# HpWang-whu/YOHO

Measured on AMD Instinct MI355X. Metric: keypoints/sec (5000 kp x60 rot desc+YOHO-O), higher is better.
Workload: dtype fp16x2 split (2^-22-accurate products, fp32 accumulate); 1 GPU

## Files before the change

yoho_amd/csrc/gemmf.h:

```cpp
#pragma once
#include <hip/hip_runtime.h>
#include <type_traits>
#include "common.h"

namespace yoho {

typedef float floatx16 __attribute__((ext_vector_type(16)));
typedef float floatx4 __attribute__((ext_vector_type(4)));
typedef unsigned uintx4 __attribute__((ext_vector_type(4)));
typedef _Float16 halfx8 __attribute__((ext_vector_type(8)));
typedef const __attribute__((address_space(1))) void* gptr_t;
typedef __attribute__((address_space(3))) void* lptr_t;

constexpr int FG_STAGE = 32768;
constexpr int FG_LDS = 4 * FG_STAGE;

static const int FG_ORD_D[NIR_ORD] = {5, 4, 3, 3, 1};
static const int FG_ORD_R[NIR_ORD] = {4, 3, 1, 2, 0};
static const int FG_IR_BASE[5] = {0, 1, 10, 19, 35};
static const int FG_IR_D[5] = {1, 3, 3, 4, 5};

struct FGemmArgs {
    const char* A;
    const char* B;
    const float* bias;
    const float* res;
    float* out;
    long long a_off[NIR_ORD], b_off[NIR_ORD];
    int NT[NIR_ORD], MT[NIR_ORD], rot[NIR_ORD];
    int dim[NIR_ORD], qbase[NIR_ORD];
    int cin, cout, kppad, nT32;
    float descale;
    int* rflag;
    const unsigned* amax;
};

template <int I, int N, typename Fn>
__device__ __forceinline__ void sfor(Fn&& f) {
    if constexpr (I < N) {
        f(std::integral_constant<int, I>{});
        sfor<I + 1, N>(f);
    }
}

__device__ __forceinline__ floatx16 mfma_h(uintx4 a, uintx4 b, floatx16 c) {
    union { uintx4 u; halfx8 h; } ca, cb;
    ca.u = a; cb.u = b;
    return __builtin_amdgcn_mfma_f32_32x32x16_f16(ca.h, cb.h, c, 0, 0, 0);
}

__device__ __forceinline__ const char* uniform_ptr(const char* p) {
    const unsigned long long v = reinterpret_cast<unsigned long long>(p);
    const unsigned lo = __builtin_amdgcn_readfirstlane((unsigned)v), hi = __builtin_amdgcn_readfirstlane((unsigned)(v >> 32));
    return reinterpret_cast<const char*>(((unsigned long long)hi << 32) | lo);
}

template <int MI, int NJ>
__device__ __forceinline__ void zero_acc(floatx16 (&acc)[MI][NJ]) {
#pragma unroll
    for (int i = 0; i < MI; ++i)
#pragma unroll
        for (int j = 0; j < NJ; ++j)
#pragma unroll
            for (int e = 0; e < 16; ++e) acc[i][j][e] = 0.f;
}

__device__ __forceinline__ bool fg3_map(const FGemmArgs& a, int xcd, int slot, int& t, int& local, int& r) {
    int start = 0;
    for (int u = 0; u < NIR_ORD; ++u) {
        const int ru = (xcd + a.rot[u]) & 7;
        const int cnt = a.NT[u] > ru ? ((a.NT[u] - 1 - ru) / 8 + 1) * a.MT[u] : 0;
        if (slot < start + cnt) { t = u; local = slot - start; r = ru; return true; }
        start += cnt;
    }
    return false;
}

inline int fgemm_grid(const FGemmArgs& a, int per_tile) {
    int tot = 0;
    for (int x = 0; x < 8; ++x) {
        int n = 0;
        for (int t = 0; t < NIR_ORD; ++t) {
            const int r = (x + a.rot[t]) & 7;
            if (a.NT[t] > r) n += ((a.NT[t] - 1 - r) / 8 + 1) * a.MT[t] * per_tile;
        }
        tot = n > tot ? n : tot;
    }
    return 8 * tot;
}

enum { F2_NOSTORE = 0x100, F2_MIX = 0x200, F2_ST_SC1 = 0x400, F2_ST_NT = 0x800, F2_SPARSE4 = 0x1000, F2_SPARSE16 = 0x2000, F2_K32 = 0x4000 };

__device__ __forceinline__ size_t slab_off(int tile32, int q, int cout8, int o, int half, int kp32) {
    return (((((size_t)tile32 * G + q) * cout8 + (o >> 3)) * 2 + half) * TILE + kp32) * 4;
}

template <int MI, int NJ>
__device__ __forceinline__ void residual_start(floatx16 (&acc)[MI][NJ], int row0, int kp0, int jidx, int d, int qbase, const float* res, float descale,
                                               int cout, int nT32, int lane) {
    const float inv = 1.f / descale;
    const int half = lane >> 5, kp32 = lane & 31, cout8 = cout >> 3;
#pragma unroll
    for (int bi = 0; bi < NJ; ++bi) {
        const int tile32 = (kp0 >> 5) + bi;
#pragma unroll
        for (int ai = 0; ai < MI; ++ai) {
            const int rowb = row0 + ai * 32;
            const int iidx = rowb / cout, o0 = rowb - iidx * cout;
            const bool ok = tile32 < nT32 && iidx < d;
            const int q = qbase + iidx * d + jidx;
#pragma unroll
            for (int q4 = 0; q4 < 4; ++q4) {
                const size_t off = slab_off(tile32, q, cout8, o0 + q4 * 8 + half * 4, half, kp32);
                const floatx4 v = *reinterpret_cast<const floatx4*>(res + (ok ? off : 0)) * (ok ? inv : 0.f);
                acc[ai][bi][4 * q4 + 0] = v.x; acc[ai][bi][4 * q4 + 1] = v.y;
                acc[ai][bi][4 * q4 + 2] = v.z; acc[ai][bi][4 * q4 + 3] = v.w;
            }
        }
    }
}

template <int MI, int NJ>
__device__ __forceinline__ void coef_epilogue(const floatx16 (&acc)[MI][NJ], int row0, int kp0, int jidx, int d, int qbase, float* out, const float* bias,
                                              float descale, int cout, int nT32, int* rflag, int lane, int flags) {
    const int half = lane >> 5, kp32 = lane & 31, cout8 = cout >> 3;
    unsigned top = 0u;
#ifdef YOHO_EXPERIMENTS
    if ((flags & F2_SPARSE4) && (blockIdx.x >> 3) % 4 != 0) flags |= F2_NOSTORE;
    if ((flags & F2_SPARSE16) && (blockIdx.x >> 3) % 16 != 0) flags |= F2_NOSTORE;
    const __amdgpu_buffer_rsrc_t orsrc = __builtin_amdgcn_make_buffer_rsrc(out, 0, 0x7FFFFFFF, 0x00020000);
#endif
#pragma unroll
    for (int bi = 0; bi < NJ; ++bi) {
        const int tile32 = (kp0 >> 5) + bi;
        if (tile32 >= nT32) continue;
#pragma unroll
        for (int ai = 0; ai < MI; ++ai) {
            const int rowb = row0 + ai * 32;
            const int iidx = rowb / cout, o0 = rowb - iidx * cout;
            if (iidx >= d) continue;
            const int q = qbase + iidx * d + jidx;
#pragma unroll
            for (int q4 = 0; q4 < 4; ++q4) {
                const int o = o0 + q4 * 8 + half * 4;
                floatx4 val;
                val.x = acc[ai][bi][4 * q4 + 0]; val.y = acc[ai][bi][4 * q4 + 1];
                val.z = acc[ai][bi][4 * q4 + 2]; val.w = acc[ai][bi][4 * q4 + 3];
                val *= descale;
                if (d == 1) val += *reinterpret_cast<const floatx4*>(bias + o) * 7.745966692414834f;
                const size_t off = slab_off(tile32, q, cout8, o, half, kp32);
#ifdef YOHO_EXPERIMENTS
                if (flags & F2_ST_SC1) __builtin_amdgcn_raw_buffer_store_b128(__builtin_bit_cast(uintx4, val), orsrc, (int)(off * 4), 0, 16);
                else if (flags & F2_ST_NT) __builtin_amdgcn_raw_buffer_store_b128(__builtin_bit_cast(uintx4, val), orsrc, (int)(off * 4), 0, 2);
                else if (!(flags & F2_NOSTORE))
#endif
                *reinterpret_cast<floatx4*>(out + off) = val;
                top = max(max(top, __float_as_uint(val.x) & 0x7FFFFFFFu), __float_as_uint(val.y) & 0x7FFFFFFFu);
                top = max(max(top, __float_as_uint(val.z) & 0x7FFFFFFFu), __float_as_uint(val.w) & 0x7FFFFFFFu);
            }
        }
    }
    note_range_bits(rflag, top, FP16_MAX / HF_ASCALE);
}

__device__ __forceinline__ floatx4 mfma_h16(uintx4 a, uintx4 b, floatx4 c) {
    union { uintx4 u; halfx8 h; } ca, cb;
    ca.u = a; cb.u = b;
    return __builtin_amdgcn_mfma_f32_16x16x32_f16(ca.h, cb.h, c, 0, 0, 0);
}

inline bool fgemm_layer_k32(const FGemmArgs& a) { return a.cin >= 256 && a.cin % 64 == 0 && a.cout >= 256; }

template <int NJ, typename Extra>
__device__ __forceinline__ void row_products32(floatx4 (&accrow)[NJ], const uintx4& al, const uintx4& ah, const uintx4 (&bh)[NJ], const uintx4 (&bl)[NJ],
                                               Extra&& extra) {
    sfor<0, 3 * NJ>([&](auto mc) {
        constexpr int m = decltype(mc)::value, j = m % NJ, p = m / NJ;
        accrow[j] = mfma_h16(p == 0 ? al : ah, p == 1 ? bl[j] : bh[j], accrow[j]);
        __builtin_amdgcn_sched_barrier(0);
        extra(mc);
        __builtin_amdgcn_sched_barrier(0);
    });
}

template <int LOB, int MI, int NJ>
__device__ __forceinline__ void stage32_plain(floatx4 (&acc)[MI][NJ], const char* pa, const char* pb) {
    uintx4 bh[NJ], bl[NJ], al[2], ah[2];
#pragma unroll
    for (int j = 0; j < NJ; ++j) {
        bh[j] = *reinterpret_cast<const uintx4*>(pb + j * 256);
        bl[j] = *reinterpret_cast<const uintx4*>(pb + LOB + j * 256);
    }
    al[0] = *reinterpret_cast<const uintx4*>(pa + 16384);
    ah[0] = *reinterpret_cast<const uintx4*>(pa);
    sfor<0, MI>([&](auto ic) {
        constexpr int i = decltype(ic)::value;
        if constexpr (i + 1 < MI) {
            al[(i + 1) & 1] = *reinterpret_cast<const uintx4*>(pa + 16384 + (i + 1) * 256);
            ah[(i + 1) & 1] = *reinterpret_cast<const uintx4*>(pa + (i + 1) * 256);
        }
        row_products32(acc[i], al[i & 1], ah[i & 1], bh, bl, [](auto) {});
    });
}

template <int MI, int NJ>
__device__ __forceinline__ void zero_acc(floatx4 (&acc)[MI][NJ]) {
#pragma unroll
    for (int i = 0; i < MI; ++i)
#pragma unroll
        for (int j = 0; j < NJ; ++j) acc[i][j] = floatx4{0.f, 0.f, 0.f, 0.f};
}

template <bool TO_SLAB>
__device__ __forceinline__ void swap_rows16(floatx4& x, floatx4& y) {
    typedef unsigned uintx2 __attribute__((ext_vector_type(2)));
#pragma unroll
    for (int e = 0; e < 4; ++e) {
        uintx2 r = {__float_as_uint(x[e]), __float_as_uint(y[e])};
        if constexpr (TO_SLAB) {
            r = __builtin_amdgcn_permlane16_swap(r.x, r.y, false, false);
            r = __builtin_amdgcn_permlane32_swap(r.x, r.y, false, false);
        } else {
            r = __builtin_amdgcn_permlane32_swap(r.x, r.y, false, false);
            r = __builtin_amdgcn_permlane16_swap(r.x, r.y, false, false);
        }
        x[e] = __uint_as_float(r.x); y[e] = __uint_as_float(r.y);
    }
}

template <int MI, int NJ>
__device__ __forceinline__ void residual_start(floatx4 (&acc)[MI][NJ], int row0, int kp0, int jidx, int d, int qbase, const float* res, float descale,
                                               int cout, int nT32, int lane) {
    static_assert(NJ % 2 == 0, "pairs of 16-column tiles");
    const float inv = 1.f / descale;
    const int half = lane >> 5, kp32 = lane & 31, cout8 = cout >> 3;
#pragma unroll
    for (int bi = 0; bi < NJ; bi += 2) {
        const int tile32 = (kp0 >> 5) + (bi >> 1);
#pragma unroll
        for (int ai = 0; ai < MI; ++ai) {
            const int rowb = row0 + ai * 16;
            const int iidx = rowb / cout, o0 = rowb - iidx * cout;
            const bool ok = tile32 < nT32 && iidx < d;
            const int q = qbase + iidx * d + jidx;
            const size_t off0 = slab_off(tile32, q, cout8, o0 + half * 4, half, kp32), off1 = slab_off(tile32, q, cout8, o0 + 8 + half * 4, half, kp32);
            acc[ai][bi] = *reinterpret_cast<const floatx4*>(res + (ok ? off0 : 0)) * (ok ? inv : 0.f);
            acc[ai][bi + 1] = *reinterpret_cast<const floatx4*>(res + (ok ? off1 : 0)) * (ok ? inv : 0.f);
            swap_rows16<false>(acc[ai][bi], acc[ai][bi + 1]);
        }
    }
}

template <int MI, int NJ>
__device__ __forceinline__ void coef_epilogue(const floatx4 (&acc)[MI][NJ], int row0, int kp0, int jidx, int d, int qbase, float* out, const float* bias,
                                              float descale, int cout, int nT32, int* rflag, int lane, int flags) {
    static_assert(NJ % 2 == 0, "pairs of 16-column tiles");
    const int half = lane >> 5, kp32 = lane & 31, cout8 = cout >> 3;
    unsigned top = 0u;
#pragma unroll
    for (int bi = 0; bi < NJ; bi += 2) {
        const int tile32 = (kp0 >> 5) + (bi >> 1);
        if (tile32 >= nT32) continue;
#pragma unroll
        for (int ai = 0; ai < MI; ++ai) {
            const int rowb = row0 + ai * 16;
            const int iidx = rowb / cout, o0 = rowb - iidx * cout;
            if (iidx >= d) continue;
            const int q = qbase + iidx * d + jidx;
            floatx4 v[2] = {acc[ai][bi], acc[ai][bi + 1]};
            swap_rows16<true>(v[0], v[1]);
#pragma unroll
            for (int h8 = 0; h8 < 2; ++h8) {
                const int o = o0 + h8 * 8 + half * 4;
                floatx4 val = v[h8] * descale;
                if (d == 1) val += *reinterpret_cast<const floatx4*>(bias + o) * 7.745966692414834f;
#ifdef YOHO_EXPERIMENTS
                if (!(flags & F2_NOSTORE))
#endif
                *reinterpret_cast<floatx4*>(out + slab_off(tile32, q, cout8, o, half, kp32)) = val;
                top = max(max(top, __float_as_uint(val.x) & 0x7FFFFFFFu), __float_as_uint(val.y) & 0x7FFFFFFFu);
                top = max(max(top, __float_as_uint(val.z) & 0x7FFFFFFFu), __float_as_uint(val.w) & 0x7FFFFFFFu);
            }
        }
    }
    note_range_bits(rflag, top, FP16_MAX / HF_ASCALE);
}

void fgemm_fill_args(FGemmArgs& a, const Layer& L, const char* Bplanes, int kppad, int nT32, const float* res, float* out, int* rflag);
int launch_fgemm2(const FGemmArgs& a, int flags, hipStream_t s);
int launch_fgemm3(const FGemmArgs& a, int flags, hipStream_t s);
int fgemm2_init();

}
```

yoho_amd/csrc/gemmf.hip:

```cpp
#include <hip/hip_runtime.h>
#include <hip/hip_fp16.h>
#include <type_traits>
#include <vector>
#include <cmath>
#include <cstring>
#include <cstdlib>

#include "common.h"
#include "gemmf.h"

namespace yoho {

struct Frags {
    uintx4 ah[4], al[4], bh[4], bl[4];
};

template <int SUB, int R>
__device__ __forceinline__ void read_frag(const char* pa, const char* pb, Frags& f) {
    constexpr int t = R & 3;
    if constexpr (R < 4) f.al[t] = *reinterpret_cast<const uintx4*>(pa + (2 + SUB) * 8192 + t * 512);
    else if constexpr (R < 8) f.bh[t] = *reinterpret_cast<const uintx4*>(pb + (0 + SUB) * 8192 + t * 512);
    else if constexpr (R < 12) f.ah[t] = *reinterpret_cast<const uintx4*>(pa + (0 + SUB) * 8192 + t * 512);
    else f.bl[t] = *reinterpret_cast<const uintx4*>(pb + (2 + SUB) * 8192 + t * 512);
}

template <int SUB>
__device__ __forceinline__ void read_frags(const char* pa, const char* pb, Frags& f) {
    sfor<0, 16>([&](auto rc) { read_frag<SUB, decltype(rc)::value>(pa, pb, f); });
}

template <int U>
__device__ __forceinline__ void stage_unit(const char* srcA, const char* srcB, char* dst, int w, int lane16) {
    constexpr int p = U & 7;
    const int blk = p * 4 + w;
    const char* src = (U < 8 ? srcA : srcB) + blk * 1024;
    char* d = dst + (U < 8 ? 0 : FG_STAGE) + blk * 1024;
    __builtin_amdgcn_global_load_lds((gptr_t)(src + lane16), (lptr_t)d, 16, 0, 0);
}

__device__ __forceinline__ void stage_tile(const char* src, char* dst, int w, int lane) {
#pragma unroll
    for (int p = 0; p < 8; ++p) {
        const int blk = p * 4 + w;
        __builtin_amdgcn_global_load_lds((gptr_t)(src + blk * 1024 + lane * 16), (lptr_t)(dst + blk * 1024), 16, 0, 0);
    }
}

template <int RSUB, bool DMA>
__device__ __forceinline__ void substep(const Frags& f, floatx16 (&acc)[4][4], const char* ra, const char* rb, Frags& nf,
                                        const char* srcA, const char* srcB, char* dmadst, int w, int lane16) {
    sfor<0, 16>([&](auto gc) {
        constexpr int g = decltype(gc)::value;
        acc[g >> 2][g & 3] = mfma_h(f.al[g >> 2], f.bh[g & 3], acc[g >> 2][g & 3]);
        read_frag<RSUB, g>(ra, rb, nf);
        __builtin_amdgcn_sched_barrier(0);
    });
    sfor<0, 16>([&](auto gc) {
        constexpr int g = decltype(gc)::value;
        acc[g >> 2][g & 3] = mfma_h(f.ah[g >> 2], f.bl[g & 3], acc[g >> 2][g & 3]);
        if constexpr (DMA) {
            stage_unit<g>(srcA, srcB, dmadst, w, lane16);
            __builtin_amdgcn_sched_barrier(0);
        }
    });
    __builtin_amdgcn_sched_barrier(0);
    sfor<0, 16>([&](auto gc) {
        constexpr int g = decltype(gc)::value;
        acc[g >> 2][g & 3] = mfma_h(f.ah[g >> 2], f.bh[g & 3], acc[g >> 2][g & 3]);
    });
    __builtin_amdgcn_sched_barrier(0);
}

__global__ __launch_bounds__(256, 1) void fgemm_kernel(FGemmArgs a, int flags) {
    extern __shared__ __attribute__((aligned(16))) char smem[];
    const int tid = threadIdx.x, lane = tid & 63;
    const int w = __builtin_amdgcn_readfirstlane(tid >> 6);
    int t = 0, local = 0, r = 0;
    if (!fg3_map(a, blockIdx.x & 7, blockIdx.x >> 3, t, local, r)) return;
    const int d = a.dim[t];
    const int MT = a.MT[t], KS = d * a.cin / 32;
    const int cg = local / MT, mtile = local - cg * MT;
    const int ntile = r + 8 * cg;
    const char* Ag = a.A + a.a_off[t] + (size_t)mtile * KS * FG_STAGE;
    const char* Bg = a.B + a.b_off[t] + (size_t)ntile * KS * FG_STAGE;
    const int wm = w >> 1, wn = w & 1;
    const int lane16 = lane * 16;
    const int row0 = mtile * 256 + wm * 128;
    const int col0 = ntile * 256 + wn * 128;

    floatx16 acc[4][4];
    zero_acc(acc);

    const int lane_a = (lane >> 5) * 4096 + (wm * 128 + (lane & 31)) * 16;
    const int lane_b = FG_STAGE + (lane >> 5) * 4096 + (wn * 128 + (lane & 31)) * 16;

    stage_tile(Ag, smem, w, lane);
    stage_tile(Bg, smem + FG_STAGE, w, lane);
    if (KS > 1) {
        stage_tile(Ag + FG_STAGE, smem + 2 * FG_STAGE, w, lane);
        stage_tile(Bg + FG_STAGE, smem + 3 * FG_STAGE, w, lane);
    }
    if ((flags & EPI_RES) && row0 < d * a.cout) residual_start(acc, row0, col0 % a.kppad, col0 / a.kppad, d, a.qbase[t], a.res, a.descale, a.cout, a.nT32, lane);
    asm volatile("s_waitcnt vmcnt(0)" ::: "memory");
    __syncthreads();

    if (row0 >= d * a.cout) {
        for (int s = 0; s < KS; ++s) {
            asm volatile("s_waitcnt vmcnt(0)" ::: "memory");
            __syncthreads();
            const int s2 = s + 2 < KS ? s + 2 : KS - 1;
            char* cur = smem + (s & 1) * (2 * FG_STAGE);
            stage_tile(Ag + (size_t)s2 * FG_STAGE, cur, w, lane);
            stage_tile(Bg + (size_t)s2 * FG_STAGE, cur + FG_STAGE, w, lane);
        }
        asm volatile("s_waitcnt vmcnt(0)" ::: "memory");
        return;
    }
    Frags P, Q;
    read_frags<0>(smem + lane_a, smem + lane_b, P);
    for (int s = 0; s < KS; ++s) {
        char* cur = smem + (s & 1) * (2 * FG_STAGE);
        char* nxt = smem + ((s + 1) & 1) * (2 * FG_STAGE);
        substep<1, false>(P, acc, cur + lane_a, cur + lane_b, Q, nullptr, nullptr, nullptr, w, lane16);
        asm volatile("s_waitcnt vmcnt(0) lgkmcnt(0)" ::: "memory");
        __syncthreads();
        __builtin_amdgcn_sched_barrier(0);
        const int s2 = s + 2 < KS ? s + 2 : KS - 1;
        substep<0, true>(Q, acc, nxt + lane_a, nxt + lane_b, P, uniform_ptr(Ag + (size_t)s2 * FG_STAGE), uniform_ptr(Bg + (size_t)s2 * FG_STAGE),
                              cur, w, lane16);
    }
    asm volatile("s_waitcnt vmcnt(0)" ::: "memory");

    coef_epilogue(acc, row0, col0 % a.kppad, col0 / a.kppad, d, a.qbase[t], a.out, a.bias, a.descale, a.cout, a.nT32, a.rflag, lane, flags);
}

__global__ __launch_bounds__(256, 1) void fgemmk_kernel(FGemmArgs a, int flags) {
    extern __shared__ __attribute__((aligned(16))) char smem[];
    const int tid = threadIdx.x, lane = tid & 63;
    const int w = __builtin_amdgcn_readfirstlane(tid >> 6);
    int t = 0, local = 0, r = 0;
    if (!fg3_map(a, blockIdx.x & 7, blockIdx.x >> 3, t, local, r)) return;
    const int d = a.dim[t];
    const int MT = a.MT[t], KS = d * a.cin / 32;
    const int cg = local / MT, mtile = local - cg * MT;
    const int ntile = r + 8 * cg;
    const char* Ag = a.A + a.a_off[t] + (size_t)mtile * KS * FG_STAGE;
    const char* Bg = a.B + a.b_off[t] + (size_t)ntile * KS * FG_STAGE;
    const int wm = w >> 1, wn = w & 1;
    const int row0 = mtile * 256 + wm * 128, col0 = ntile * 256 + wn * 128;
    const bool rows_live = row0 < d * a.cout;
    const int lane_a = (lane >> 4) * 4096 + (wm * 128 + (lane & 15)) * 16;
    const int lane_b = FG_STAGE + (lane >> 4) * 4096 + (wn * 128 + (lane & 15)) * 16;

    floatx4 acc[8][8];
    zero_acc(acc);
    stage_tile(Ag, smem, w, lane);
    stage_tile(Bg, smem + FG_STAGE, w, lane);
    if (KS > 1) {
        stage_tile(Ag + FG_STAGE, smem + 2 * FG_STAGE, w, lane);
        stage_tile(Bg + FG_STAGE, smem + 3 * FG_STAGE, w, lane);
    }
    if ((flags & EPI_RES) && rows_live) residual_start(acc, row0, col0 % a.kppad, col0 / a.kppad, d, a.qbase[t], a.res, a.descale, a.cout, a.nT32, lane);
    asm volatile("s_waitcnt vmcnt(0)" ::: "memory");
    __syncthreads();
    for (int s = 0; s < KS; ++s) {
        char* cur = smem + (s & 1) * (2 * FG_STAGE);
        if (rows_live) stage32_plain<FG_STAGE / 2>(acc, cur + lane_a, cur + lane_b);
        asm volatile("s_waitcnt vmcnt(0) lgkmcnt(0)" ::: "memory");
        __syncthreads();
        __builtin_amdgcn_sched_barrier(0);
        if (s + 2 < KS) {
            stage_tile(uniform_ptr(Ag + (size_t)(s + 2) * FG_STAGE), cur, w, lane);
            stage_tile(uniform_ptr(Bg + (size_t)(s + 2) * FG_STAGE), cur + FG_STAGE, w, lane);
        }
    }
    if (rows_live) coef_epilogue(acc, row0, col0 % a.kppad, col0 / a.kppad, d, a.qbase[t], a.out, a.bias, a.descale, a.cout, a.nT32, a.rflag, lane, flags);
}

int fgemm_init() {
    HIPCHK(hipFuncSetAttribute(reinterpret_cast<const void*>(&fgemm_kernel), hipFuncAttributeMaxDynamicSharedMemorySize, FG_LDS));
    HIPCHK(hipFuncSetAttribute(reinterpret_cast<const void*>(&fgemmk_kernel), hipFuncAttributeMaxDynamicSharedMemorySize, FG_LDS));
    if (int rc = cgemm_init()) return rc;
    return fgemm2_init();
}

static long long pack_off(int t, int rows, int kdim) {
    long long off = 0;
    for (int u = 0; u < t; ++u) off += (long long)((FG_ORD_D[u] * rows + 255) / 256) * (FG_ORD_D[u] * kdim / 32) * FG_STAGE;
    return off;
}

size_t fgemm_planes_bytes(int kppad, int cin) { return (size_t)pack_off(NIR_ORD, kppad, cin); }

void fgemm_qinfo(int* qi ) {
    for (int t = 0; t < NIR_ORD; ++t) {
        const int r = FG_ORD_R[t], d = FG_IR_D[r];
        for (int m = 0; m < d; ++m)
            for (int j = 0; j < d; ++j) {
                int* p = qi + (FG_IR_BASE[r] + m * d + j) * 4;
                p[0] = t; p[1] = m; p[2] = j; p[3] = d;
            }
    }
}
void fgemm_plane_offsets(int kppad, int cin, long long* off ) {
    for (int t = 0; t < NIR_ORD; ++t) off[t] = pack_off(t, kppad, cin);
}

static inline unsigned short half_bits_h(float x) {
    const _Float16 h = (_Float16)x;
    unsigned short u;
    std::memcpy(&u, &h, 2);
    return u;
}

static unsigned char e4m3_bits(float x) {
    const unsigned sgn = std::signbit(x) ? 0x80u : 0u;
    const float a = std::fabs(x);
    if (!(a == a)) return 0x7F;
    if (a >= 464.f) return (unsigned char)(sgn | 0x7E);
    if (a < std::ldexp(1.f, -6)) {
        const int r = (int)std::nearbyint(std::ldexp(a, 9));
        return (unsigned char)(sgn | (r == 8 ? 0x08 : r));
    }
    int e;
    (void)std::frexp(a, &e);
    int r = (int)std::nearbyint(std::ldexp(a, 3 - (e - 1)));
    if (r == 16) { r = 8; ++e; }
    const int E = e - 1 + 7;
    if (E > 15 || (E == 15 && r - 8 > 6)) return (unsigned char)(sgn | 0x7E);
    return (unsigned char)(sgn | (E << 3) | (r - 8));
}
static inline float half_value_h(unsigned short u) {
    _Float16 h;
    std::memcpy(&h, &u, 2);
    return (float)h;
}

static inline size_t apack_index(int row, int k, int KS) {
    const int mtile = row >> 8, rr = row & 255, ks = k >> 5, sub = (k >> 4) & 1, kg = (k >> 3) & 1, e = k & 7;
    return ((size_t)mtile * KS + ks) * (FG_STAGE / 2) + ((size_t)(sub * 2 + kg) * 256 + rr) * 8 + e;
}
static inline void put_split(unsigned short* pack, size_t idx, float x) {
    const _Float16 hi = (_Float16)x;
    pack[idx] = half_bits_h(x);
    pack[idx + 8192] = half_bits_h(x - (float)hi);
}
static void fp8_correction_planes(const std::vector<unsigned short>& out, std::vector<unsigned short>& out8) {
    out8 = out;
    const size_t nblk = out.size() / (FG_STAGE / 2);
    for (size_t b = 0; b < nblk; ++b) {
        const unsigned short* src = out.data() + b * (FG_STAGE / 2);
        unsigned char* dst = reinterpret_cast<unsigned char*>(out8.data() + b * (FG_STAGE / 2) + 8192);
        for (int u = 0; u < 1024; ++u)
            for (int e = 0; e < 8; ++e) {
                dst[u * 16 + e] = e4m3_bits(half_value_h(src[u * 8 + e]) * 0.25f);
                dst[u * 16 + 8 + e] = e4m3_bits(half_value_h(src[8192 + u * 8 + e]) * 512.f);
            }
    }
}

int pack_fgemm_weights(const FourierBasis& fb, const float* W, int cin, int cout, std::vector<unsigned short>& out, float* descale,
                       std::vector<unsigned short>* out8) {
    if ((cout % 256 && cout != 32) || cin % 32) return -1;
    std::vector<float> what((size_t)60 * cout * cin);
    std::vector<double> coef(60 * NTAP);
    for (int r = 0; r < 5; ++r) {
        const int d = FG_IR_D[r];
        for (int i = 0; i < d; ++i)
            for (int m = 0; m < d; ++m)
                for (int k = 0; k < NTAP; ++k) coef[(FG_IR_BASE[r] + i * d + m) * NTAP + k] = fb.rho[r][fb.n0[k]][m * d + i];
    }
    float wmax = 0.f;
    for (int f = 0; f < 60; ++f)
        for (int o = 0; o < cout; ++o)
            for (int c = 0; c < cin; ++c) {
                const float* wk = W + ((size_t)o * cin + c) * NTAP;
                double acc = 0.0;
                for (int k = 0; k < NTAP; ++k) acc += (double)wk[k] * coef[f * NTAP + k];
                const float v = (float)acc;
                what[((size_t)f * cout + o) * cin + c] = v;
                wmax = std::fmax(wmax, std::fabs(v));
            }
    int ex = 0;
    if (wmax > 0.f && std::isfinite(wmax)) (void)std::frexp(wmax, &ex);
    const float wscale = std::ldexp(1.f, 10 - ex);
    *descale = 1.f / (wscale * HF_ASCALE);
    out.assign((size_t)pack_off(NIR_ORD, cout, cin) / 2, 0);
    for (int t = 0; t < NIR_ORD; ++t) {
        const int r = FG_ORD_R[t], d = FG_IR_D[r];
        unsigned short* base = out.data() + pack_off(t, cout, cin) / 2;
        for (int i = 0; i < d; ++i)
            for (int o = 0; o < cout; ++o)
                for (int m = 0; m < d; ++m) {
                    const float* src = &what[((size_t)(FG_IR_BASE[r] + i * d + m) * cout + o) * cin];
                    for (int c = 0; c < cin; ++c) put_split(base, apack_index(i * cout + o, m * cin + c, d * cin / 32), src[c] * wscale);
                }
    }
    if (out8) fp8_correction_planes(out, *out8);
    return 0;
}

int pack_cgemm_weights(const float* W, int cin, int cout, int ntaps, std::vector<unsigned short>& out, float* descale, std::vector<unsigned short>& out8) {
    if (cout % 256 || cin % 32) return -1;
    float wmax = 0.f;
    for (size_t i = 0; i < (size_t)cout * cin * ntaps; ++i) wmax = std::fmax(wmax, std::fabs(W[i]));
    int ex = 0;
    if (wmax > 0.f && std::isfinite(wmax)) (void)std::frexp(wmax, &ex);
    const float wscale = std::ldexp(1.f, 10 - ex);
    *descale = 1.f / (wscale * H2_ASCALE);
    const int KS = ntaps * cin / 32;
    out.assign((size_t)(cout / 256) * KS * (FG_STAGE / 2), 0);
    for (int o = 0; o < cout; ++o)
        for (int tap = 0; tap < ntaps; ++tap)
            for (int c = 0; c < cin; ++c) put_split(out.data(), apack_index(o, tap * cin + c, KS), W[((size_t)o * cin + c) * ntaps + tap] * wscale);
    fp8_correction_planes(out, out8);
    return 0;
}

void fgemm_fill_args(FGemmArgs& a, const Layer& L, const char* Bplanes, int kppad, int nT32, const float* res, float* out, int* rflag) {
    a.rflag = rflag; a.amax = nullptr;
    a.A = reinterpret_cast<const char*>(L.wpg); a.B = Bplanes; a.bias = L.bias; a.res = res; a.out = out;
    a.cin = L.cin; a.cout = L.cout; a.kppad = kppad; a.nT32 = nT32; a.descale = L.wpg_descale;
    static const int ROT[NIR_ORD] = {0, 0, 4, 4, 2};
    for (int t = 0; t < NIR_ORD; ++t) {
        a.a_off[t] = pack_off(t, L.cout, L.cin);
        a.b_off[t] = pack_off(t, kppad, L.cin);
        a.MT[t] = (FG_ORD_D[t] * L.cout + 255) / 256;
        a.NT[t] = FG_ORD_D[t] * kppad / 256;
        a.rot[t] = ROT[t];
        a.dim[t] = FG_ORD_D[t];
        a.qbase[t] = FG_IR_BASE[FG_ORD_R[t]];
    }
}

int launch_fgemm(const Layer& L, const char* Bplanes, int kppad, int nT32, const float* res, float* out, int flags, hipStream_t s, int* rflag,
                 FGemmBlocking blocking, const unsigned* amax) {
    FGemmArgs a;
    fgemm_fill_args(a, L, Bplanes, kppad, nT32, res, out, rflag);
    static const int dbg_gemm1 = [] { const char* e = experiment_env("YOHO_PARTI_DEBUG"); return (e && std::strstr(e, "gemm1")) ? 1 : 0; }();
    if (dbg_gemm1) blocking = FG_TILE256_W4;
    if (blocking == FG_TILE256_W8 && amax && L.wpg8) { a.amax = amax; a.A = reinterpret_cast<const char*>(L.wpg8); }
    const char* dbg = experiment_env("YOHO_FGEMM_DEBUG");
    if (fgemm_layer_k32(a) && !a.amax && !(dbg && std::strstr(dbg, "k16"))) flags |= F2_K32;
    if (blocking == FG_TILE256_W8) return launch_fgemm3(a, flags, s);
    if (blocking != FG_TILE256_W4) return launch_fgemm2(a, flags, s);
    if (flags & F2_K32) hipLaunchKernelGGL(fgemmk_kernel, dim3(fgemm_grid(a, 1)), dim3(256), FG_LDS, s, a, flags);
    else hipLaunchKernelGGL(fgemm_kernel, dim3(fgemm_grid(a, 1)), dim3(256), FG_LDS, s, a, flags);
    HIPCHK(hipGetLastError());
    return 0;
}

}
```

yoho_amd/csrc/gemmf2.hip:

```cpp
#include <hip/hip_runtime.h>
#include <cstdlib>
#include <cstring>
#include "common.h"
#include "gemmf.h"

namespace yoho {

constexpr int F2_BUF = 24576;
constexpr int F2_LDS = 3 * F2_BUF;
constexpr int F3_BUF = 32768;
constexpr int F3_LDS = 3 * F3_BUF;

struct Frags2 {
    uintx4 ah[4], al[4], bh[2], bl[2];
};

template <int LO, int R>
__device__ __forceinline__ void read_frag2(const char* pa, const char* pb, Frags2& f) {
    if constexpr (R < 4) f.al[R] = *reinterpret_cast<const uintx4*>(pa + 8192 + R * 512);
    else if constexpr (R < 6) f.bh[R - 4] = *reinterpret_cast<const uintx4*>(pb + (R - 4) * 512);
    else if constexpr (R < 10) f.ah[R - 6] = *reinterpret_cast<const uintx4*>(pa + (R - 6) * 512);
    else f.bl[R - 10] = *reinterpret_cast<const uintx4*>(pb + LO + (R - 10) * 512);
}
template <int LO>
__device__ __forceinline__ void read_frags2(const char* pa, const char* pb, Frags2& f) {
    sfor<0, 12>([&](auto rc) { read_frag2<LO, decltype(rc)::value>(pa, pb, f); });
}

struct Dma2 {
    static constexpr int NP = 6, LO = 4096;
    int la, lb, w;
    __device__ __forceinline__ Dma2(int w_, int lane) : la(w_ * 1024 + lane * 16), lb((w_ >> 1) * 4096 + (w_ & 1) * 1024 + lane * 16), w(w_) {}
    template <int U>
    __device__ __forceinline__ void piece(const char* srcA, const char* srcB, char* buf) const {
        if constexpr (U < 4) {
            constexpr int plane = U >> 1, kg = U & 1;
            __builtin_amdgcn_global_load_lds((gptr_t)(srcA + plane * 16384 + kg * 4096 + la), (lptr_t)(buf + plane * 8192 + kg * 4096 + w * 1024), 16, 0, 0);
        } else {
            constexpr int plane = U - 4;
            __builtin_amdgcn_global_load_lds((gptr_t)(srcB + plane * 16384 + lb), (lptr_t)(buf + 16384 + plane * 4096 + (w >> 1) * 2048 + (w & 1) * 1024), 16, 0, 0);
        }
    }
};
struct Dma3 {
    static constexpr int NP = 4, LO = 8192;
    int la, ldst;
    __device__ __forceinline__ Dma3(int w8, int lane) : la(w8 * 1024 + lane * 16), ldst(w8 * 1024) {}
    template <int U>
    __device__ __forceinline__ void piece(const char* srcA, const char* srcB, char* buf) const {
        constexpr int plane = U & 1;
        if constexpr (U < 2) __builtin_amdgcn_global_load_lds((gptr_t)(srcA + plane * 16384 + la), (lptr_t)(buf + plane * 8192 + ldst), 16, 0, 0);
        else __builtin_amdgcn_global_load_lds((gptr_t)(srcB + plane * 16384 + la), (lptr_t)(buf + 16384 + plane * 8192 + ldst), 16, 0, 0);
    }
};
template <typename Dma>
__device__ __forceinline__ void dma_step(const Dma& dm, const char* srcA, const char* srcB, char* buf) {
    sfor<0, Dma::NP>([&](auto uc) { dm.template piece<decltype(uc)::value>(srcA, srcB, buf); });
}

template <bool DMA, typename Dma>
__device__ __forceinline__ void step2(const Dma& dm, const Frags2& f, floatx16 (&acc)[4][2], const char* ra, const char* rb, Frags2& nf,
                                      const char* srcA, const char* srcB, char* dmabuf) {
    sfor<0, 8>([&](auto gc) {
        constexpr int g = decltype(gc)::value;
        acc[g >> 1][g & 1] = mfma_h(f.al[g >> 1], f.bh[g & 1], acc[g >> 1][g & 1]);
        read_frag2<Dma::LO, g>(ra, rb, nf);
        __builtin_amdgcn_sched_barrier(0);
    });
    sfor<0, 8>([&](auto gc) {
        constexpr int g = decltype(gc)::value;
        acc[g >> 1][g & 1] = mfma_h(f.ah[g >> 1], f.bl[g & 1], acc[g >> 1][g & 1]);
        if constexpr (g < 4) read_frag2<Dma::LO, 8 + g>(ra, rb, nf);
        else if constexpr (DMA) dm.template piece<g - 4>(srcA, srcB, dmabuf);
        __builtin_amdgcn_sched_barrier(0);
    });
    sfor<0, 8>([&](auto gc) {
        constexpr int g = decltype(gc)::value;
        acc[g >> 1][g & 1] = mfma_h(f.ah[g >> 1], f.bh[g & 1], acc[g >> 1][g & 1]);
        if constexpr (DMA && 4 + g < Dma::NP) dm.template piece<4 + g>(srcA, srcB, dmabuf);
        __builtin_amdgcn_sched_barrier(0);
    });
}

__host__ __device__ inline bool fg2_map(const FGemmArgs& a, int xcd, int slot, bool contiguous, int& t, int& local, int& r) {
    int cnt[NIR_ORD], ru[NIR_ORD];
    for (int u = 0; u < NIR_ORD; ++u) {
        ru[u] = (xcd + a.rot[u]) & 7;
        cnt[u] = a.NT[u] > ru[u] ? ((a.NT[u] - 1 - ru[u]) / 8 + 1) * a.MT[u] * 2 : 0;
    }
    const int L = cnt[0], S = cnt[1] + cnt[2] + cnt[3] + cnt[4];
    int list, idx;
    if (contiguous) { list = slot < L ? 0 : 1; idx = slot < L ? slot : slot - L; }
    else {
        const int P = L < S ? L : S;
        if (slot < 2 * P) { list = slot & 1; idx = slot >> 1; }
        else { list = L > S ? 0 : 1; idx = P + (slot - 2 * P); }
    }
    if (list == 0) {
        if (idx >= L) return false;
        t = 0; local = idx; r = ru[0];
        return true;
    }
    for (int u = 1; u < NIR_ORD; ++u) {
        if (idx < cnt[u]) { t = u; local = idx; r = ru[u]; return true; }
        idx -= cnt[u];
    }
    return false;
}

__device__ __forceinline__ size_t step_off(int ks) { return (size_t)(ks >> 1) * FG_STAGE + (size_t)(ks & 1) * 8192; }

template <int BUF, typename Dma>
__device__ __forceinline__ void ring_prologue(int KT, Dma&& dma) {
    dma(0, 0);
    dma(1, BUF);
    if (KT > 2) dma(2, 2 * BUF);
}

template <int BUF, int INFLIGHT, typename F, typename Step>
__device__ __forceinline__ void ring_pipelined(char* smem, const char* Ag, const char* Bg, int KT, int lane_a, int lane_b, F& P, Step&& step) {
    F Q;
    asm volatile("s_waitcnt lgkmcnt(0)" ::: "memory");
    __builtin_amdgcn_s_barrier();
    __builtin_amdgcn_sched_barrier(0);
    int cur = 0, nxt = BUF;
    int s = 0;
    auto run = [&](auto dma, const F& f, F& nf) {
        if constexpr (decltype(dma)::value) {
            step(dma, f, nf, smem + nxt + lane_a, smem + nxt + lane_b, uniform_ptr(Ag + step_off(s + 3)), uniform_ptr(Bg + step_off(s + 3)), smem + cur);
            asm volatile("s_waitcnt vmcnt(%0) lgkmcnt(0)" ::"n"(INFLIGHT) : "memory");
        } else {
            step(dma, f, nf, smem + nxt + lane_a, smem + nxt + lane_b, nullptr, nullptr, nullptr);
            asm volatile("s_waitcnt vmcnt(0) lgkmcnt(0)" ::: "memory");
        }
        __builtin_amdgcn_s_barrier();
        __builtin_amdgcn_sched_barrier(0);
        cur = nxt; nxt = nxt == 2 * BUF ? 0 : nxt + BUF; ++s;
    };
    constexpr std::true_type dma;
    constexpr std::false_type nodma;
    while (s + 4 < KT) {
        run(dma, P, Q);
        run(dma, Q, P);
    }
    if (KT >= 4) {
        run(dma, P, Q);
        run(nodma, Q, P);
    }
    run(nodma, P, Q);
    step(nodma, Q, P, smem + cur + lane_a, smem + cur + lane_b, nullptr, nullptr, nullptr);
}

template <int BUF, typename Dma>
__device__ __forceinline__ void ring_pipelined_idle(int KT, Dma&& dma) {
    __builtin_amdgcn_s_barrier();
    for (int s = 0; s + 1 < KT; ++s) {
        if (s + 3 < KT) dma(s + 3, (s % 3) * BUF);
        asm volatile("s_waitcnt vmcnt(0)" ::: "memory");
        __builtin_amdgcn_s_barrier();
    }
}

__global__ __launch_bounds__(256, 2) void fgemm2_kernel(FGemmArgs a, int flags) {
    extern __shared__ __attribute__((aligned(16))) char smem[];
    const int tid = threadIdx.x, lane = tid & 63;
    const int w = __builtin_amdgcn_readfirstlane(tid >> 6);
    int t = 0, local = 0, r = 0;
    if (!fg2_map(a, blockIdx.x & 7, blockIdx.x >> 3, (flags & F2_MIX) == 0, t, local, r)) return;
    const int d = a.dim[t];
    const int MT = a.MT[t], KS = d * a.cin / 32, KT = 2 * KS;
    const int nh = local & 1, pair = local >> 1;
    const int cg = pair / MT, mtile = pair - cg * MT;
    const int ntile = r + 8 * cg;
    const char* Ag = a.A + a.a_off[t] + (size_t)mtile * KS * FG_STAGE;
    const char* Bg = a.B + a.b_off[t] + (size_t)ntile * KS * FG_STAGE + nh * 2048;
    const int wm = w >> 1, wn = w & 1;
    const Dma2 dm(w, lane);
    const int lane_a = (lane >> 5) * 4096 + (wm * 128 + (lane & 31)) * 16;
    const int lane_b = 16384 + (lane >> 5) * 2048 + (wn * 64 + (lane & 31)) * 16;

    floatx16 acc[4][2];
    zero_acc(acc);
    auto dma = [&](int st, int buf) { dma_step(dm, Ag + step_off(st), Bg + step_off(st), smem + buf); };
    ring_prologue<F2_BUF>(KT, dma);
    const int row0 = mtile * 256 + wm * 128, colbase = ntile * 256 + nh * 128 + wn * 64;
    const bool rows_live = row0 < d * a.cout;
    const int jidx = colbase / a.kppad, kp0 = colbase - jidx * a.kppad, qbase = a.qbase[t];
    if ((flags & EPI_RES) && rows_live) residual_start(acc, row0, kp0, jidx, d, qbase, a.res, a.descale, a.cout, a.nT32, lane);
    asm volatile("s_waitcnt vmcnt(0)" ::: "memory");
    __builtin_amdgcn_s_barrier();
    if (!rows_live) return ring_pipelined_idle<F2_BUF>(KT, dma);

    Frags2 P;
    read_frags2<Dma2::LO>(smem + lane_a, smem + lane_b, P);
    ring_pipelined<F2_BUF, 6>(smem, Ag, Bg, KT, lane_a, lane_b, P,
        [&](auto dmac, const Frags2& f, Frags2& nf, const char* ra, const char* rb, const char* srcA, const char* srcB, char* buf) {
            step2<decltype(dmac)::value>(dm, f, acc, ra, rb, nf, srcA, srcB, buf);
        });
    coef_epilogue(acc, row0, kp0, jidx, d, qbase, a.out, a.bias, a.descale, a.cout, a.nT32, a.rflag, lane, flags);
}

struct Wave3 {
    int wm, wn, nh, lane_a, lane_b;
    Dma3 dm;
    __device__ __forceinline__ Wave3(int w8, int lane) : wm((w8 & 3) >> 1), wn(w8 & 1), nh(w8 >> 2), dm(w8, lane) {
        lane_a = (lane >> 5) * 4096 + (wm * 128 + (lane & 31)) * 16;
        lane_b = 16384 + (lane >> 5) * 4096 + (nh * 128 + wn * 64 + (lane & 31)) * 16;
    }
};

__global__ __launch_bounds__(512, 2) void fgemm3_kernel(FGemmArgs a, int flags) {
    extern __shared__ __attribute__((aligned(16))) char smem[];
    const int tid = threadIdx.x, lane = tid & 63;
    const Wave3 wv(__builtin_amdgcn_readfirstlane(tid >> 6), lane);
    int t = 0, local = 0, r = 0;
    if (!fg3_map(a, blockIdx.x & 7, blockIdx.x >> 3, t, local, r)) return;
    const int d = a.dim[t];
    const int MT = a.MT[t], KS = d * a.cin / 32, KT = 2 * KS;
    const int cg = local / MT, mtile = local - cg * MT;
    const int ntile = r + 8 * cg;
    const char* Ag = a.A + a.a_off[t] + (size_t)mtile * KS * FG_STAGE;
    const char* Bg = a.B + a.b_off[t] + (size_t)ntile * KS * FG_STAGE;

    floatx16 acc[4][2];
    zero_acc(acc);
    auto dma = [&](int st, int buf) { dma_step(wv.dm, Ag + step_off(st), Bg + step_off(st), smem + buf); };
    ring_prologue<F3_BUF>(KT, dma);
    const int row0 = mtile * 256 + wv.wm * 128, colbase = ntile * 256 + wv.nh * 128 + wv.wn * 64;
    const bool rows_live = row0 < d * a.cout;
    const int jidx = colbase / a.kppad, kp0 = colbase - jidx * a.kppad, qbase = a.qbase[t];
    if ((flags & EPI_RES) && rows_live) residual_start(acc, row0, kp0, jidx, d, qbase, a.res, a.descale, a.cout, a.nT32, lane);
    asm volatile("s_waitcnt vmcnt(0)" ::: "memory");
    __builtin_amdgcn_s_barrier();
    if (!rows_live) return ring_pipelined_idle<F3_BUF>(KT, dma);

    Frags2 P;
    read_frags2<Dma3::LO>(smem + wv.lane_a, smem + wv.lane_b, P);
    ring_pipelined<F3_BUF, 4>(smem, Ag, Bg, KT, wv.lane_a, wv.lane_b, P,
        [&](auto dmac, const Frags2& f, Frags2& nf, const char* ra, const char* rb, const char* srcA, const char* srcB, char* buf) {
            step2<decltype(dmac)::value>(wv.dm, f, acc, ra, rb, nf, srcA, srcB, buf);
        });
    coef_epilogue(acc, row0, kp0, jidx, d, qbase, a.out, a.bias, a.descale, a.cout, a.nT32, a.rflag, lane, flags);
}

constexpr int F3K_BUF = 2 * FG_STAGE;
constexpr int F3K_LDS = 2 * F3K_BUF;

struct Dma3k {
    static constexpr int NP = 8;
    int la, ldst;
    __device__ __forceinline__ Dma3k(int w8, int lane) : la(w8 * 1024 + lane * 16), ldst(w8 * 1024) {}
    template <int U>
    __device__ __forceinline__ void piece(const char* srcA, const char* srcB, char* buf) const {
        constexpr int q = (U & 3) * 8192;
        if constexpr (U < 4) __builtin_amdgcn_global_load_lds((gptr_t)(srcA + q + la), (lptr_t)(buf + q + ldst), 16, 0, 0);
        else __builtin_amdgcn_global_load_lds((gptr_t)(srcB + q + la), (lptr_t)(buf + FG_STAGE + q + ldst), 16, 0, 0);
    }
};
struct FragsA32 { uintx4 al, ah; };
struct FragsB32 { uintx4 bh[4], bl[4]; };

template <int R>
__device__ __forceinline__ void read_open32(const char* pa, const char* pb, FragsA32& a0, FragsB32& b) {
    if constexpr (R == 0) a0.al = *reinterpret_cast<const uintx4*>(pa + 16384);
    else if constexpr (R < 5) b.bh[R - 1] = *reinterpret_cast<const uintx4*>(pb + (R - 1) * 256);
    else if constexpr (R == 5) a0.ah = *reinterpret_cast<const uintx4*>(pa);
    else b.bl[R - 6] = *reinterpret_cast<const uintx4*>(pb + 16384 + (R - 6) * 256);
}

template <bool DMA>
__device__ __forceinline__ void step32(const Dma3k& dm, floatx4 (&acc)[8][4], FragsA32 (&fa)[2], const FragsB32& b, FragsB32& nb, const char* pa,
                                       const char* npa, const char* npb, const char* srcA, const char* srcB, char* dmabuf) {
    sfor<0, 7>([&](auto ic) {
        constexpr int i = decltype(ic)::value;
        row_products32(acc[i], fa[i & 1].al, fa[i & 1].ah, b.bh, b.bl, [&](auto mc) {
            constexpr int m = decltype(mc)::value;
            if constexpr (m == 1) fa[(i + 1) & 1].al = *reinterpret_cast<const uintx4*>(pa + 16384 + (i + 1) * 256);
            if constexpr (m == 2) fa[(i + 1) & 1].ah = *reinterpret_cast<const uintx4*>(pa + (i + 1) * 256);
        });
    });
    asm volatile("s_waitcnt vmcnt(0) lgkmcnt(0)" ::: "memory");
    __builtin_amdgcn_s_barrier();
    __builtin_amdgcn_sched_barrier(0);
    row_products32(acc[7], fa[1].al, fa[1].ah, b.bh, b.bl, [&](auto mc) {
        constexpr int m = decltype(mc)::value;
        if constexpr (m < 5) {
            read_open32<2 * m>(npa, npb, fa[0], nb);
            read_open32<2 * m + 1>(npa, npb, fa[0], nb);
        }
        if constexpr (DMA && m >= 4) dm.template piece<m - 4>(srcA, srcB, dmabuf);
    });
}

__global__ __launch_bounds__(512, 2) void fgemm3k_kernel(FGemmArgs a, int flags) {
    extern __shared__ __attribute__((aligned(16))) char smem[];
    const int tid = threadIdx.x, lane = tid & 63;
    const int w8 = __builtin_amdgcn_readfirstlane(tid >> 6);
    int t = 0, local = 0, r = 0;
    if (!fg3_map(a, blockIdx.x & 7, blockIdx.x >> 3, t, local, r)) return;
    const int d = a.dim[t];
    const int MT = a.MT[t], KS = d * a.cin / 32;
    const int cg = local / MT, mtile = local - cg * MT;
    const int ntile = r + 8 * cg;
    const char* Ag = a.A + a.a_off[t] + (size_t)mtile * KS * FG_STAGE;
    const char* Bg = a.B + a.b_off[t] + (size_t)ntile * KS * FG_STAGE;
    const int wm = (w8 & 3) >> 1, wn = w8 & 1, nh = w8 >> 2;
    const Dma3k dm(w8, lane);
    const int lane_a = (lane >> 4) * 4096 + (wm * 128 + (lane & 15)) * 16;
    const int lane_b = FG_STAGE + (lane >> 4) * 4096 + (nh * 128 + wn * 64 + (lane & 15)) * 16;

    floatx4 acc[8][4];
    zero_acc(acc);
    auto dma = [&](int st, int buf) {
        const char* sa = uniform_ptr(Ag + (size_t)st * FG_STAGE);
        const char* sb = uniform_ptr(Bg + (size_t)st * FG_STAGE);
        sfor<0, Dma3k::NP>([&](auto uc) { dm.template piece<decltype(uc)::value>(sa, sb, smem + buf); });
    };
    dma(0, 0);
    if (KS > 1) dma(1, F3K_BUF);
    const int row0 = mtile * 256 + wm * 128, colbase = ntile * 256 + nh * 128 + wn * 64;
    const bool rows_live = row0 < d * a.cout;
    const int jidx = colbase / a.kppad, kp0 = colbase - jidx * a.kppad, qbase = a.qbase[t];
    if ((flags & EPI_RES) && rows_live) residual_start(acc, row0, kp0, jidx, d, qbase, a.res, a.descale, a.cout, a.nT32, lane);
    asm volatile("s_waitcnt vmcnt(0)" ::: "memory");
    __builtin_amdgcn_s_barrier();
    if (!rows_live) {
        for (int s = 0; s < KS; ++s) {
            asm volatile("s_waitcnt vmcnt(0)" ::: "memory");
            __builtin_amdgcn_s_barrier();
            if (s + 2 < KS) dma(s + 2, (s & 1) * F3K_BUF);
        }
        asm volatile("s_waitcnt vmcnt(0)" ::: "memory");
        return;
    }

    FragsA32 fa[2];
    FragsB32 P, Q;
    sfor<0, 10>([&](auto rc) { read_open32<decltype(rc)::value>(smem + lane_a, smem + lane_b, fa[0], P); });
    int s = 0, cur = 0;
    auto run = [&](auto dmac, const FragsB32& b, FragsB32& nb) {
        const int nxt = cur ^ F3K_BUF;
        if constexpr (decltype(dmac)::value)
            step32<true>(dm, acc, fa, b, nb, smem + cur + lane_a, smem + nxt + lane_a, smem + nxt + lane_b, uniform_ptr(Ag + (size_t)(s + 2) * FG_STAGE),
                         uniform_ptr(Bg + (size_t)(s + 2) * FG_STAGE), smem + cur);
        else
            step32<false>(dm, acc, fa, b, nb, smem + cur + lane_a, smem + nxt + lane_a, smem + nxt + lane_b, nullptr, nullptr, nullptr);
        cur = nxt; ++s;
    };
    constexpr std::true_type dmay;
    constexpr std::false_type dman;
    while (s + 2 < KS) {
        run(dmay, P, Q);
        run(dmay, Q, P);
    }
    run(dman, P, Q);
    run(dman, Q, P);
    coef_epilogue(acc, row0, kp0, jidx, d, qbase, a.out, a.bias, a.descale, a.cout, a.nT32, a.rflag, lane, flags);
}

constexpr int F2K_BUF = FG_STAGE + FG_STAGE / 2;
constexpr int F2K_LDS = 2 * F2K_BUF;

__global__ __launch_bounds__(256, 1) void fgemm2k_kernel(FGemmArgs a, int flags) {
    extern __shared__ __attribute__((aligned(16))) char smem[];
    const int tid = threadIdx.x, lane = tid & 63;
    const int w = __builtin_amdgcn_readfirstlane(tid >> 6);
    int t = 0, local = 0, r = 0;
    if (!fg2_map(a, blockIdx.x & 7, blockIdx.x >> 3, (flags & F2_MIX) == 0, t, local, r)) return;
    const int d = a.dim[t];
    const int MT = a.MT[t], KS = d * a.cin / 32;
    const int nh = local & 1, pair = local >> 1;
    const int cg = pair / MT, mtile = pair - cg * MT;
    const int ntile = r + 8 * cg;
    const char* Ag = a.A + a.a_off[t] + (size_t)mtile * KS * FG_STAGE;
    const char* Bg = a.B + a.b_off[t] + (size_t)ntile * KS * FG_STAGE + nh * 2048;
    const int wm = w >> 1, wn = w & 1;
    const int lane_a = (lane >> 4) * 4096 + (wm * 128 + (lane & 15)) * 16;
    const int lane_b = FG_STAGE + (lane >> 4) * 2048 + (wn * 64 + (lane & 15)) * 16;

    floatx4 acc[8][4];
    zero_acc(acc);
    auto dma = [&](int st, int buf) {
        const char* sa = uniform_ptr(Ag + (size_t)st * FG_STAGE) + lane * 16;
        const char* sb = uniform_ptr(Bg + (size_t)st * FG_STAGE) + lane * 16;
#pragma unroll
        for (int k = 0; k < 8; ++k) __builtin_amdgcn_global_load_lds((gptr_t)(sa + (k * 4 + w) * 1024), (lptr_t)(smem + buf + (k * 4 + w) * 1024), 16, 0, 0);
#pragma unroll
        for (int k = 0; k < 4; ++k) {
            const int pb = w * 4 + k, u = pb >> 1, part = pb & 1;
            __builtin_amdgcn_global_load_lds((gptr_t)(sb + u * 4096 + part * 1024), (lptr_t)(smem + buf + FG_STAGE + u * 2048 + part * 1024), 16, 0, 0);
        }
    };
    dma(0, 0);
    if (KS > 1) dma(1, F2K_BUF);
    const int row0 = mtile * 256 + wm * 128, colbase = ntile * 256 + nh * 128 + wn * 64;
    const bool rows_live = row0 < d * a.cout;
    const int jidx = colbase / a.kppad, kp0 = colbase - jidx * a.kppad, qbase = a.qbase[t];
    if ((flags & EPI_RES) && rows_live) residual_start(acc, row0, kp0, jidx, d, qbase, a.res, a.descale, a.cout, a.nT32, lane);
    asm volatile("s_waitcnt vmcnt(0)" ::: "memory");
    __builtin_amdgcn_s_barrier();
    for (int s = 0; s < KS; ++s) {
        const int cur = (s & 1) * F2K_BUF;
        if (rows_live) stage32_plain<FG_STAGE / 4>(acc, smem + cur + lane_a, smem + cur + lane_b);
        asm volatile("s_waitcnt vmcnt(0) lgkmcnt(0)" ::: "memory");
        __builtin_amdgcn_s_barrier();
        __builtin_amdgcn_sched_barrier(0);
        if (s + 2 < KS) dma(s + 2, cur);
    }
    if (rows_live) coef_epilogue(acc, row0, kp0, jidx, d, qbase, a.out, a.bias, a.descale, a.cout, a.nT32, a.rflag, lane, flags);
}

typedef int intx8 __attribute__((ext_vector_type(8)));
typedef short shortx2 __attribute__((ext_vector_type(2)));
typedef _Float16 halfx2 __attribute__((ext_vector_type(2)));
struct Frags8 {
    intx8 a[4], b[2];
};
struct C8Scales {
    float ah = 4.f, al = 4.f / 2048.f, bh = 1.f, bl = 1.f;
    int mfma_b = 127;
    C8Scales() = default;
    __device__ __forceinline__ explicit C8Scales(const unsigned* amax) {
        const unsigned amax_bits = __builtin_amdgcn_readfirstlane(*amax);
        int kexp = (int)(amax_bits >> 23) - 127 - 7;
        kexp = kexp < -60 ? -60 : (kexp > 9 ? 9 : kexp);
        bh = __uint_as_float((unsigned)(kexp + 127) << 23); bl = __uint_as_float((unsigned)(kexp - 11 + 127) << 23);
        mfma_b = 127 + kexp;
    }
};
struct Int2 { int x, y; };
__device__ __forceinline__ Int2 frag_to_fp8(uintx4 f, float scale) {
    union { unsigned u; halfx2 h; } p0, p1, p2, p3;
    p0.u = f[0]; p1.u = f[1]; p2.u = f[2]; p3.u = f[3];
    shortx2 r = {0, 0}, q = {0, 0};
    r = __builtin_amdgcn_cvt_scalef32_pk_fp8_f16(r, p0.h, scale, false);
    r = __builtin_amdgcn_cvt_scalef32_pk_fp8_f16(r, p1.h, scale, true);
    q = __builtin_amdgcn_cvt_scalef32_pk_fp8_f16(q, p2.h, scale, false);
    q = __builtin_amdgcn_cvt_scalef32_pk_fp8_f16(q, p3.h, scale, true);
    Int2 o;
    __builtin_memcpy(&o.x, &r, 4);
    __builtin_memcpy(&o.y, &q, 4);
    return o;
}

template <int PAR>
__device__ __forceinline__ void step3c(const Frags2& f, floatx16 (&acc)[4][2], Frags8& c8, const C8Scales& sc) {
#pragma unroll
    for (int i = 0; i < 4; ++i)
#pragma unroll
        for (int j = 0; j < 2; ++j) acc[i][j] = mfma_h(f.ah[i], f.bh[j], acc[i][j]);
#pragma unroll
    for (int i = 0; i < 4; ++i)
#pragma unroll
        for (int e = 0; e < 4; ++e) c8.a[i][4 * PAR + e] = (int)f.al[i][e];
#pragma unroll
    for (int j = 0; j < 2; ++j) {
        const Int2 l = frag_to_fp8(f.bl[j], sc.bl), h = frag_to_fp8(f.bh[j], sc.bh);
        c8.b[j][4 * PAR] = l.x; c8.b[j][4 * PAR + 1] = l.y; c8.b[j][4 * PAR + 2] = h.x; c8.b[j][4 * PAR + 3] = h.y;
    }
    if constexpr (PAR == 1) {
#pragma unroll
        for (int i = 0; i < 4; ++i)
#pragma unroll
            for (int j = 0; j < 2; ++j)
                acc[i][j] = __builtin_amdgcn_mfma_scale_f32_32x32x64_f8f6f4(c8.a[i], c8.b[j], acc[i][j], 0, 0, 0, 127 + 2 - 11, 0, sc.mfma_b);
    }
}

template <bool FP8, typename BSrc>
__device__ __forceinline__ void ring_plain(floatx16 (&acc)[4][2], char* smem, const Wave3& wv, const char* Ag, BSrc&& bsrc, int KT, bool rows_live,
                                           const C8Scales& sc) {
    Frags8 c8;
    if constexpr (FP8) {
#pragma unroll
        for (int i = 0; i < 4; ++i)
#pragma unroll
            for (int e = 0; e < 8; ++e) c8.a[i][e] = 0;
#pragma unroll
        for (int j = 0; j < 2; ++j)
#pragma unroll
            for (int e = 0; e < 8; ++e) c8.b[j][e] = 0;
    }
    int cur = 0, stg = 2 * F3_BUF;
    int s = 0;
    auto stage = [&] {
        const int s2 = s + 2 < KT ? s + 2 : KT - 1;
        dma_step(wv.dm, uniform_ptr(Ag + step_off(s2)), uniform_ptr(bsrc(s2)), smem + stg);
    };
    auto rotate = [&] { stg = cur; cur = cur == 2 * F3_BUF ? 0 : cur + F3_BUF; ++s; };
    auto one_step = [&](auto parity) {
        asm volatile("s_waitcnt vmcnt(4) lgkmcnt(0)" ::: "memory");
        __builtin_amdgcn_s_barrier();
        __builtin_amdgcn_sched_barrier(0);
        stage();
        Frags2 f;
        read_frags2<Dma3::LO>(smem + cur + wv.lane_a, smem + cur + wv.lane_b, f);
        if constexpr (FP8) step3c<decltype(parity)::value>(f, acc, c8, sc);
        else {
#pragma unroll
            for (int i = 0; i < 4; ++i)
#pragma unroll
                for (int j = 0; j < 2; ++j) acc[i][j] = mfma_h(f.al[i], f.bh[j], acc[i][j]);
#pragma unroll
            for (int i = 0; i < 4; ++i)
#pragma unroll
                for (int j = 0; j < 2; ++j) acc[i][j] = mfma_h(f.ah[i], f.bl[j], acc[i][j]);
#pragma unroll
            for (int i = 0; i < 4; ++i)
#pragma unroll
                for (int j = 0; j < 2; ++j) acc[i][j] = mfma_h(f.ah[i], f.bh[j], acc[i][j]);
        }
        rotate();
    };
    if (rows_live) {
        for (int it = 0; it < KT; it += 2) {
            one_step(std::integral_constant<int, 0>{});
            one_step(std::integral_constant<int, 1>{});
        }
    } else {
        for (int it = 0; it < KT; ++it) {
            asm volatile("s_waitcnt vmcnt(4) lgkmcnt(0)" ::: "memory");
            __builtin_amdgcn_s_barrier();
            stage();
            rotate();
        }
    }
    asm volatile("s_waitcnt vmcnt(0)" ::: "memory");
}

__global__ __launch_bounds__(512, 2) void fgemm3c_kernel(FGemmArgs a, int flags) {
    extern __shared__ __attribute__((aligned(16))) char smem[];
    const int tid = threadIdx.x, lane = tid & 63;
    const Wave3 wv(__builtin_amdgcn_readfirstlane(tid >> 6), lane);
    int t = 0, local = 0, r = 0;
    if (!fg3_map(a, blockIdx.x & 7, blockIdx.x >> 3, t, local, r)) return;
    const int d = a.dim[t];
    const int MT = a.MT[t], KS = d * a.cin / 32, KT = 2 * KS;
    const int cg = local / MT, mtile = local - cg * MT;
    const int ntile = r + 8 * cg;
    const char* Ag = a.A + a.a_off[t] + (size_t)mtile * KS * FG_STAGE;
    const char* Bg = a.B + a.b_off[t] + (size_t)ntile * KS * FG_STAGE;

    floatx16 acc[4][2];
    zero_acc(acc);
    const C8Scales sc(a.amax);
    dma_step(wv.dm, Ag, Bg, smem);
    dma_step(wv.dm, Ag + step_off(1), Bg + step_off(1), smem + F3_BUF);
    const int row0 = mtile * 256 + wv.wm * 128, colbase = ntile * 256 + wv.nh * 128 + wv.wn * 64;
    const bool rows_live = row0 < d * a.cout;
    const int jidx = colbase / a.kppad, kp0 = colbase - jidx * a.kppad, qbase = a.qbase[t];
    if ((flags & EPI_RES) && rows_live) residual_start(acc, row0, kp0, jidx, d, qbase, a.res, a.descale, a.cout, a.nT32, lane);
    asm volatile("s_waitcnt vmcnt(0)" ::: "memory");
    __builtin_amdgcn_s_barrier();

    ring_plain<true>(acc, smem, wv, Ag, [&](int s) { return Bg + step_off(s); }, KT, rows_live, sc);
    if (rows_live) coef_epilogue(acc, row0, kp0, jidx, d, qbase, a.out, a.bias, a.descale, a.cout, a.nT32, a.rflag, lane, flags);
}

struct CGemmArgs {
    const char* A;
    const char* B;
    const float* bias;
    const float* bn_s;
    const float* bn_t;
    char* out;
    int NTm, MT, KSt, ntap, nj, nslot, c8out, nT32, nTiles16;
    float descale;
    int* rflag;
    const unsigned* amax;
    unsigned char slot[13 * 13];
    unsigned char outg[16];
};

__device__ __forceinline__ void cg_split_pair(float x0, float x1, unsigned& hi, unsigned& lo) {
    typedef float f2 __attribute__((ext_vector_type(2)));
    f2 x;
    x.x = x0; x.y = x1;
    const halfx2 h = __builtin_convertvector(x, halfx2);
    const f2 r = x - __builtin_convertvector(h, f2);
    const halfx2 l = __builtin_convertvector(r, halfx2);
    __builtin_memcpy(&hi, &h, 4);
    __builtin_memcpy(&lo, &l, 4);
}

template <bool FP8>
__global__ __launch_bounds__(512, 2) void cgemm_kernel(CGemmArgs a) {
    extern __shared__ __attribute__((aligned(16))) char smem[];
    __shared__ int tapoff[16];
    const int tid = threadIdx.x, lane = tid & 63;
    const Wave3 wv(__builtin_amdgcn_readfirstlane(tid >> 6), lane);
    const int xcd = blockIdx.x & 7, slot_ = blockIdx.x >> 3;
    const int ct = xcd + 8 * (slot_ / a.MT), mtile = slot_ % a.MT;
    if (ct >= a.nj * a.NTm) return;
    const int j = ct / a.NTm, mt = ct - j * a.NTm;
    const int SPT = 2 * a.KSt;
    const int KT = a.ntap * SPT;
    if (tid < 16) tapoff[tid] = tid < a.ntap ? (int)a.slot[j * 13 + tid] : 0;
    const char* Ag = a.A + (size_t)mtile * (KT / 2) * FG_STAGE;
    const char* Bt = a.B + (size_t)mt * a.nslot * a.KSt * FG_STAGE;
    __syncthreads();
    auto bsrc = [&](int s) -> const char* {
        const int tap = s / SPT, within = s - tap * SPT;
        const int sl = __builtin_amdgcn_readfirstlane(tapoff[tap]);
        return Bt + (size_t)sl * a.KSt * FG_STAGE + step_off(within);
    };

    floatx16 acc[4][2];
    zero_acc(acc);
    C8Scales sc;
    if constexpr (FP8) sc = C8Scales(a.amax);
    dma_step(wv.dm, Ag, uniform_ptr(bsrc(0)), smem);
    dma_step(wv.dm, Ag + step_off(1), uniform_ptr(bsrc(1)), smem + F3_BUF);
    asm volatile("s_waitcnt vmcnt(0)" ::: "memory");
    __builtin_amdgcn_s_barrier();

    ring_plain<FP8>(acc, smem, wv, Ag, bsrc, KT, true, sc);

    const int half = lane >> 5, c32 = lane & 31;
    const int g = a.outg[j];
    unsigned top = 0u;
#pragma unroll
    for (int bi = 0; bi < 2; ++bi) {
        const int m = mt * 256 + wv.nh * 128 + wv.wn * 64 + bi * 32 + c32;
        if ((m >> 5) >= a.nT32 || (m >> 4) >= a.nTiles16) continue;
#pragma unroll
        for (int ai = 0; ai < 4; ++ai) {
#pragma unroll
            for (int q4 = 0; q4 < 4; ++q4) {
                const int o = mtile * 256 + wv.wm * 128 + ai * 32 + q4 * 8 + half * 4;
                const floatx4 b4 = *reinterpret_cast<const floatx4*>(a.bias + o);
                const floatx4 s4 = *reinterpret_cast<const floatx4*>(a.bn_s + o);
                const floatx4 t4 = *reinterpret_cast<const floatx4*>(a.bn_t + o);
                float y[4];
#pragma unroll
                for (int e = 0; e < 4; ++e) {
                    const float v = acc[ai][bi][4 * q4 + e] * a.descale + b4[e];
                    y[e] = fmaxf(v * s4[e] + t4[e], 0.f) * H2_ASCALE;
                    top = max(top, __float_as_uint(y[e]) & 0x7FFFFFFFu);
                }
                unsigned h0, l0, h1, l1;
                cg_split_pair(y[0], y[1], h0, l0);
                cg_split_pair(y[2], y[3], h1, l1);
                char* dst = a.out + (((size_t)(m >> 4) * a.c8out + (o >> 3)) * 2) * 15360 + g * 256 + (m & 15) * 16 + half * 8;
                *reinterpret_cast<uint2*>(dst) = uint2{h0, h1};
                *reinterpret_cast<uint2*>(dst + 15360) = uint2{l0, l1};
            }
        }
    }
    note_range_bits(a.rflag, top, FP16_MAX);
}

__global__ __launch_bounds__(512, 2) void cgemmk_kernel(CGemmArgs a) {
    extern __shared__ __attribute__((aligned(16))) char smem[];
    __shared__ int tapoff[16];
    const int tid = threadIdx.x, lane = tid & 63;
    const int w8 = __builtin_amdgcn_readfirstlane(tid >> 6);
    const int xcd = blockIdx.x & 7, slot_ = blockIdx.x >> 3;
    const int ct = xcd + 8 * (slot_ / a.MT), mtile = slot_ % a.MT;
    if (ct >= a.nj * a.NTm) return;
    const int j = ct / a.NTm, mt = ct - j * a.NTm;
    const int KS = a.ntap * a.KSt;
    if (tid < 16) tapoff[tid] = tid < a.ntap ? (int)a.slot[j * 13 + tid] : 0;
    const char* Ag = a.A + (size_t)mtile * KS * FG_STAGE;
    const char* Bt = a.B + (size_t)mt * a.nslot * a.KSt * FG_STAGE;
    __syncthreads();
    auto bsrc = [&](int st) -> const char* {
        const int tap = st / a.KSt, cb = st - tap * a.KSt;
        const int sl = __builtin_amdgcn_readfirstlane(tapoff[tap]);
        return uniform_ptr(Bt + ((size_t)sl * a.KSt + cb) * FG_STAGE);
    };
    const int wm = (w8 & 3) >> 1, wn = w8 & 1, nh = w8 >> 2;
    const Dma3k dm(w8, lane);
    const int lane_a = (lane >> 4) * 4096 + (wm * 128 + (lane & 15)) * 16;
    const int lane_b = FG_STAGE + (lane >> 4) * 4096 + (nh * 128 + wn * 64 + (lane & 15)) * 16;

    floatx4 acc[8][4];
    zero_acc(acc);
    auto dma = [&](int st, int buf) {
        const char* sa = uniform_ptr(Ag + (size_t)st * FG_STAGE);
        const char* sb = bsrc(st);
        sfor<0, Dma3k::NP>([&](auto uc) { dm.template piece<decltype(uc)::value>(sa, sb, smem + buf); });
    };
    dma(0, 0);
    dma(1, F3K_BUF);
    asm volatile("s_waitcnt vmcnt(0)" ::: "memory");
    __builtin_amdgcn_s_barrier();

    FragsA32 fa[2];
    FragsB32 P, Q;
    sfor<0, 10>([&](auto rc) { read_open32<decltype(rc)::value>(smem + lane_a, smem + lane_b, fa[0], P); });
    int s = 0, cur = 0;
    auto run = [&](auto dmac, const FragsB32& b, FragsB32& nb) {
        const int nxt = cur ^ F3K_BUF;
        if constexpr (decltype(dmac)::value)
            step32<true>(dm, acc, fa, b, nb, smem + cur + lane_a, smem + nxt + lane_a, smem + nxt + lane_b, uniform_ptr(Ag + (size_t)(s + 2) * FG_STAGE),
                         bsrc(s + 2), smem + cur);
        else
            step32<false>(dm, acc, fa, b, nb, smem + cur + lane_a, smem + nxt + lane_a, smem + nxt + lane_b, nullptr, nullptr, nullptr);
        cur = nxt; ++s;
    };
    constexpr std::true_type dmay;
    constexpr std::false_type dman;
    while (s + 2 < KS) {
        run(dmay, P, Q);
        run(dmay, Q, P);
    }
    run(dman, P, Q);
    run(dman, Q, P);

    int etid = threadIdx.x;
    asm volatile("" : "+v"(etid));
    const int g4 = (etid >> 4) & 3, c16 = etid & 15;
    const int g = a.outg[j];
    const int col0 = mt * 256 + nh * 128 + wn * 64;
    unsigned top = 0u;
#pragma unroll
    for (int ai = 0; ai < 8; ++ai) {
        const int o = mtile * 256 + wm * 128 + ai * 16 + g4 * 4;
        const floatx4 b4 = *reinterpret_cast<const floatx4*>(a.bias + o);
        const floatx4 s4 = *reinterpret_cast<const floatx4*>(a.bn_s + o);
        const floatx4 t4 = *reinterpret_cast<const floatx4*>(a.bn_t + o);
#pragma unroll
        for (int bi = 0; bi < 4; ++bi) {
            const int m0 = col0 + bi * 16;
            if ((m0 >> 5) >= a.nT32 || (m0 >> 4) >= a.nTiles16) continue;
            float y[4];
#pragma unroll
            for (int e = 0; e < 4; ++e) {
                const float v = acc[ai][bi][e] * a.descale + b4[e];
                y[e] = fmaxf(v * s4[e] + t4[e], 0.f) * H2_ASCALE;
                top = max(top, __float_as_uint(y[e]) & 0x7FFFFFFFu);
            }
            unsigned h0, l0, h1, l1;
            cg_split_pair(y[0], y[1], h0, l0);
            cg_split_pair(y[2], y[3], h1, l1);
            char* dst = a.out + (((size_t)(m0 >> 4) * a.c8out + (o >> 3)) * 2) * 15360 + g * 256 + c16 * 16 + (g4 & 1) * 8;
            *reinterpret_cast<uint2*>(dst) = uint2{h0, h1};
            *reinterpret_cast<uint2*>(dst + 15360) = uint2{l0, l1};
        }
    }
    note_range_bits(a.rflag, top, FP16_MAX);
}

int cgemm_init() {
    HIPCHK(hipFuncSetAttribute(reinterpret_cast<const void*>(&cgemm_kernel<true>), hipFuncAttributeMaxDynamicSharedMemorySize, F3_LDS));
    HIPCHK(hipFuncSetAttribute(reinterpret_cast<const void*>(&cgemm_kernel<false>), hipFuncAttributeMaxDynamicSharedMemorySize, F3_LDS));
    HIPCHK(hipFuncSetAttribute(reinterpret_cast<const void*>(&cgemmk_kernel), hipFuncAttributeMaxDynamicSharedMemorySize, F3K_LDS));
    return 0;
}

int launch_cgemm(const Layer& L, const char* Bstages, int nslot, const unsigned char* slot, const unsigned char* outg, int nT32, int nTiles16,
                 char* out, hipStream_t s, int* rflag, const unsigned* amax) {
    const bool fp8 = amax != nullptr;
    if (!(fp8 ? L.wcg8 : L.wcg) || L.cin % 32 || L.cout % 256) { set_error("cgemm: needs the cone-GEMM weight pack, cin %% 32 == 0, cout %% 256 == 0"); return YOHO_EINVAL; }
    if (nT32 == 0) return 0;
    CGemmArgs a;
    a.A = reinterpret_cast<const char*>(fp8 ? L.wcg8 : L.wcg); a.B = Bstages; a.bias = L.bias; a.bn_s = L.bn_s; a.bn_t = L.bn_t; a.out = out;
    a.NTm = (nT32 + 7) / 8; a.MT = L.cout / 256; a.KSt = L.cin / 32; a.ntap = 13; a.nj = 13; a.nslot = nslot; a.c8out = L.cout / 8;
    a.nT32 = nT32; a.nTiles16 = nTiles16; a.descale = L.wcg_descale; a.rflag = rflag; a.amax = amax;
    std::memcpy(a.slot, slot, 169);
    std::memset(a.outg, 0, 16);
    std::memcpy(a.outg, outg, 13);
    const int CT = a.nj * a.NTm;
    const int grid = 8 * ((CT + 7) / 8) * a.MT;
    const char* dbg = experiment_env("YOHO_FGEMM_DEBUG");
    const bool k32 = !fp8 && (a.ntap * a.KSt) % 2 == 0 && !(dbg && std::strstr(dbg, "k16"));
    if (fp8) hipLaunchKernelGGL(cgemm_kernel<true>, dim3(grid), dim3(512), F3_LDS, s, a);
    else if (k32) hipLaunchKernelGGL(cgemmk_kernel, dim3(grid), dim3(512), F3K_LDS, s, a);
    else hipLaunchKernelGGL(cgemm_kernel<false>, dim3(grid), dim3(512), F3_LDS, s, a);
    HIPCHK(hipGetLastError());
    return 0;
}

struct Frags3s {
    uintx4 ah[5], al[5], bh, bl;
};

template <int R>
__device__ __forceinline__ void read_frag3s(const char* pa, const char* pb, Frags3s& f) {
    if constexpr (R < 5) f.al[R] = *reinterpret_cast<const uintx4*>(pa + 8192 + R * 512);
    else if constexpr (R == 5) f.bh = *reinterpret_cast<const uintx4*>(pb);
    else if constexpr (R < 11) f.ah[R - 6] = *reinterpret_cast<const uintx4*>(pa + (R - 6) * 512);
    else f.bl = *reinterpret_cast<const uintx4*>(pb + 8192);
}

template <bool DMA, int D>
__device__ __forceinline__ void step3s(const Frags3s& f, floatx16 (&acc)[5][1], const char* ra, const char* rb, Frags3s& nf,
                                       const char* srcA, const char* srcB, char* dmabuf, const Dma3& dm) {
    sfor<0, 5>([&](auto gc) {
        constexpr int g = decltype(gc)::value;
        if constexpr (g < D) acc[g][0] = mfma_h(f.al[g], f.bh, acc[g][0]);
        if constexpr (g < D) read_frag3s<g>(ra, rb, nf);
        if constexpr (g == 4) read_frag3s<5>(ra, rb, nf);
        __builtin_amdgcn_sched_barrier(0);
    });
    sfor<0, 5>([&](auto gc) {
        constexpr int g = decltype(gc)::value;
        if constexpr (g < D) acc[g][0] = mfma_h(f.ah[g], f.bl, acc[g][0]);
        if constexpr (g < D) read_frag3s<6 + g>(ra, rb, nf);
        if constexpr (g == 4) read_frag3s<11>(ra, rb, nf);
        __builtin_amdgcn_sched_barrier(0);
    });
    sfor<0, 5>([&](auto gc) {
        constexpr int g = decltype(gc)::value;
        if constexpr (g < D) acc[g][0] = mfma_h(f.ah[g], f.bh, acc[g][0]);
        if constexpr (DMA && g < 4) dm.template piece<g>(srcA, srcB, dmabuf);
        __builtin_amdgcn_sched_barrier(0);
    });
}

template <int D>
__device__ __forceinline__ void fgemm3s_kloop(floatx16 (&acc)[5][1], char* smem, const char* Ag, const char* Bg, int KT, const Dma3& dm, int lane_a, int lane_b) {
    Frags3s P;
    sfor<0, 12>([&](auto rc) {
        constexpr int R = decltype(rc)::value;
        if constexpr (R == 5 || R == 11 || (R < 5 && R < D) || (R > 5 && R < 11 && R - 6 < D)) read_frag3s<R>(smem + lane_a, smem + lane_b, P);
    });
    ring_pipelined<F3_BUF, 4>(smem, Ag, Bg, KT, lane_a, lane_b, P,
        [&](auto dmac, const Frags3s& f, Frags3s& nf, const char* ra, const char* rb, const char* srcA, const char* srcB, char* buf) {
            step3s<decltype(dmac)::value, D>(f, acc, ra, rb, nf, srcA, srcB, buf, dm);
        });
}

__global__ __launch_bounds__(512, 2) void fgemm3s_kernel(FGemmArgs a, int flags) {
    extern __shared__ __attribute__((aligned(16))) char smem[];
    const int tid = threadIdx.x, lane = tid & 63;
    const int w8 = __builtin_amdgcn_readfirstlane(tid >> 6);
    int t = 0, local = 0, r = 0;
    if (!fg3_map(a, blockIdx.x & 7, blockIdx.x >> 3, t, local, r)) return;
    const int d = a.dim[t];
    const int KS = d * a.cin / 32, KT = 2 * KS;
    const int ntile = r + 8 * local;
    const char* Ag = a.A + a.a_off[t];
    const char* Bg = a.B + a.b_off[t] + (size_t)ntile * KS * FG_STAGE;
    const Dma3 dm(w8, lane);
    const int lane_a = (lane >> 5) * 4096 + (lane & 31) * 16;
    const int lane_b = 16384 + (lane >> 5) * 4096 + (w8 * 32 + (lane & 31)) * 16;

    floatx16 acc[5][1];
    zero_acc(acc);
    ring_prologue<F3_BUF>(KT, [&](int st, int buf) { dma_step(dm, uniform_ptr(Ag + step_off(st)), uniform_ptr(Bg + step_off(st)), smem + buf); });
    asm volatile("s_waitcnt vmcnt(0)" ::: "memory");
    __builtin_amdgcn_s_barrier();

    switch (d) {
        case 1: fgemm3s_kloop<1>(acc, smem, Ag, Bg, KT, dm, lane_a, lane_b); break;
        case 3: fgemm3s_kloop<3>(acc, smem, Ag, Bg, KT, dm, lane_a, lane_b); break;
        case 4: fgemm3s_kloop<4>(acc, smem, Ag, Bg, KT, dm, lane_a, lane_b); break;
        default: fgemm3s_kloop<5>(acc, smem, Ag, Bg, KT, dm, lane_a, lane_b); break;
    }
    const int colbase = ntile * 256 + w8 * 32;
    const int jidx = colbase / a.kppad, kp0 = colbase - jidx * a.kppad;
    coef_epilogue(acc, 0, kp0, jidx, d, a.qbase[t], a.out, a.bias, a.descale, 32, a.nT32, a.rflag, lane, flags & F2_NOSTORE);
}

int fgemm3_init() {
    HIPCHK(hipFuncSetAttribute(reinterpret_cast<const void*>(&fgemm3_kernel), hipFuncAttributeMaxDynamicSharedMemorySize, F3_LDS));
    HIPCHK(hipFuncSetAttribute(reinterpret_cast<const void*>(&fgemm3s_kernel), hipFuncAttributeMaxDynamicSharedMemorySize, F3_LDS));
    HIPCHK(hipFuncSetAttribute(reinterpret_cast<const void*>(&fgemm3c_kernel), hipFuncAttributeMaxDynamicSharedMemorySize, F3_LDS));
    HIPCHK(hipFuncSetAttribute(reinterpret_cast<const void*>(&fgemm3k_kernel), hipFuncAttributeMaxDynamicSharedMemorySize, F3K_LDS));
    return 0;
}

int launch_fgemm3(const FGemmArgs& a, int flags, hipStream_t s) {
    if (const char* dbg = experiment_env("YOHO_FGEMM_DEBUG")) {
        if (std::strstr(dbg, "nostore")) flags |= F2_NOSTORE;
        if (std::strstr(dbg, "sc1")) flags |= F2_ST_SC1;
        if (std::strstr(dbg, "stnt")) flags |= F2_ST_NT;
    }
    const int tot = fgemm_grid(a, 1);
    static const bool small_ok = [] { const char* e = experiment_env("YOHO_FGEMM_DEBUG"); return !(e && std::strstr(e, "nosmall")); }();
    if (small_ok && a.cout == 32 && !(flags & EPI_RES)) hipLaunchKernelGGL(fgemm3s_kernel, dim3(tot), dim3(512), F3_LDS, s, a, flags);
    else if (a.amax) hipLaunchKernelGGL(fgemm3c_kernel, dim3(tot), dim3(512), F3_LDS, s, a, flags);
    else if (flags & F2_K32) hipLaunchKernelGGL(fgemm3k_kernel, dim3(tot), dim3(512), F3K_LDS, s, a, flags);
    else hipLaunchKernelGGL(fgemm3_kernel, dim3(tot), dim3(512), F3_LDS, s, a, flags);
    HIPCHK(hipGetLastError());
    return 0;
}

int fgemm2_init() {
    HIPCHK(hipFuncSetAttribute(reinterpret_cast<const void*>(&fgemm2_kernel), hipFuncAttributeMaxDynamicSharedMemorySize, F2_LDS));
    HIPCHK(hipFuncSetAttribute(reinterpret_cast<const void*>(&fgemm2k_kernel), hipFuncAttributeMaxDynamicSharedMemorySize, F2K_LDS));
    return fgemm3_init();
}

int launch_fgemm2(const FGemmArgs& a, int flags, hipStream_t s) {
    if (const char* dbg = experiment_env("YOHO_FGEMM_DEBUG")) {
        if (std::strstr(dbg, "nostore")) flags |= F2_NOSTORE;
        if (std::strstr(dbg, "mix")) flags |= F2_MIX;
        if (std::strstr(dbg, "sc1")) flags |= F2_ST_SC1;
        if (std::strstr(dbg, "nt")) flags |= F2_ST_NT;
        if (std::strstr(dbg, "sparse4")) flags |= F2_SPARSE4;
        if (std::strstr(dbg, "sparse16")) flags |= F2_SPARSE16;
    }
    if (flags & F2_K32) hipLaunchKernelGGL(fgemm2k_kernel, dim3(fgemm_grid(a, 2)), dim3(256), F2K_LDS, s, a, flags);
    else hipLaunchKernelGGL(fgemm2_kernel, dim3(fgemm_grid(a, 2)), dim3(256), F2_LDS, s, a, flags);
    HIPCHK(hipGetLastError());
    return 0;
}

}
```

yoho_amd/csrc/gft16.hip:

```cpp
#include <hip/hip_runtime.h>
#include <cstdlib>
#include <type_traits>
#include <vector>
#include <cmath>
#include <cstring>

#include "common.h"

namespace yoho {

typedef float floatx16 __attribute__((ext_vector_type(16)));
typedef float floatx2 __attribute__((ext_vector_type(2)));
typedef float floatx4 __attribute__((ext_vector_type(4)));
typedef unsigned uintx4 __attribute__((ext_vector_type(4)));
typedef _Float16 halfx8 __attribute__((ext_vector_type(8)));
typedef _Float16 halfx2 __attribute__((ext_vector_type(2)));
typedef const __attribute__((address_space(1))) void* gptr_t;
typedef __attribute__((address_space(3))) void* lptr_t;

constexpr int GB = 65536;
constexpr int G16_LDS = 2 * GB + 1024;
constexpr int G16X_MAXC = 512;
constexpr int G16X_LDS = G16_LDS + 2 * G16X_MAXC * 4;
constexpr float F_SCALE = 1024.f;

struct Gft16Args {
    const float* in;
    float* out32;
    char* planes;
    const uintx4* Ffrag;
    const float* bn_s;
    const float* bn_t;
    int nChunks, C8, B;
    float* res0;
    int nTiles16;
    long long qbase[G];
    int qstride[G];
    int* rflag;
    int drain;
    int* ctr;
    unsigned* amax;
};

__device__ __forceinline__ floatx16 mfma_hh(uintx4 a, uintx4 b, floatx16 c) {
    union { uintx4 u; halfx8 h; } ca, cb;
    ca.u = a; cb.u = b;
    return __builtin_amdgcn_mfma_f32_32x32x16_f16(ca.h, cb.h, c, 0, 0, 0);
}

__device__ __forceinline__ void split_pair(float x0, float x1, unsigned& hi, unsigned& lo) {
    floatx2 x;
    x.x = x0; x.y = x1;
    const halfx2 h = __builtin_convertvector(x, halfx2);
    const floatx2 r = x - __builtin_convertvector(h, floatx2);
    const halfx2 l = __builtin_convertvector(r, halfx2);
    __builtin_memcpy(&hi, &h, 4);
    __builtin_memcpy(&lo, &l, 4);
}
__device__ __forceinline__ void split_pair(float x0, float x1, unsigned& hi, unsigned& lo, unsigned& top) {
    top = max(max(top, __float_as_uint(x0) & 0x7FFFFFFFu), __float_as_uint(x1) & 0x7FFFFFFFu);
    split_pair(x0, x1, hi, lo);
}

__device__ __forceinline__ void stage_chunk(const float* in, int chunk, int C8, char* dst, int w, int lane) {
    const int c8 = chunk % C8, tile32 = chunk / C8;
    const char* s = reinterpret_cast<const char*>(in) + ((size_t)tile32 * G * C8 + c8) * 1024;
    const size_t rs = (size_t)C8 * 1024;
    for (int p = w; p < G; p += 4) __builtin_amdgcn_global_load_lds((gptr_t)(s + p * rs + lane * 16), (lptr_t)(dst + p * 1024), 16, 0, 0);
}

enum { G16_ACT32 = 0, G16_ACTP = 1, G16_INV = 2, G16_INVP = 3, G16_INVG = 4 };

template <int MODE>
__global__ __launch_bounds__(256, 1) void gft16_kernel(Gft16Args a) {
    constexpr bool PLANES = MODE == G16_ACTP;
    extern __shared__ __attribute__((aligned(16))) char smem[];
    const int tid = threadIdx.x, lane = tid & 63;
    const int w = __builtin_amdgcn_readfirstlane(tid >> 6);
    const int Lp = lane & 31, kg = lane >> 5;

    for (int i = tid; i < 2 * 256; i += 256) {
        const int bsel = i >> 8, j = i & 255;
        reinterpret_cast<uintx4*>(smem + bsel * GB + G * 1024)[j] = uintx4{0u, 0u, 0u, 0u};
    }
    long long* qb = reinterpret_cast<long long*>(smem + 2 * GB);
    int* qs = reinterpret_cast<int*>(smem + 2 * GB + 512);
    if (tid < G) { qb[tid] = a.qbase[tid]; qs[tid] = a.qstride[tid]; }

    uintx4 A1[2][4][2], A2[2][4][2];
#pragma unroll
    for (int rb = 0; rb < 2; ++rb)
#pragma unroll
        for (int kb = 0; kb < 4; ++kb)
#pragma unroll
            for (int pl = 0; pl < 2; ++pl) {
                A1[rb][kb][pl] = a.Ffrag[(((0 * 2 + rb) * 4 + kb) * 2 + pl) * 64 + lane];
                A2[rb][kb][pl] = a.Ffrag[(((1 * 2 + rb) * 4 + kb) * 2 + pl) * 64 + lane];
            }

    unsigned top = 0u;
    int chunk = blockIdx.x;
    if (chunk < a.nChunks) stage_chunk(a.in, chunk, a.C8, smem, w, lane);
    for (int it = 0; chunk < a.nChunks; chunk += gridDim.x, ++it) {
        char* cur = smem + (it & 1) * GB;
        asm volatile("s_waitcnt vmcnt(0)" ::: "memory");
        __syncthreads();
        const int next = chunk + gridDim.x;
        if (next < a.nChunks) stage_chunk(a.in, next, a.C8, smem + ((it + 1) & 1) * GB, w, lane);
        const int c8 = chunk % a.C8, tile32 = chunk / a.C8;

        floatx16 acc[2][2];
#pragma unroll
        for (int rb = 0; rb < 2; ++rb)
#pragma unroll
            for (int f = 0; f < 2; ++f)
#pragma unroll
                for (int r = 0; r < 16; ++r) acc[rb][f][r] = 0.f;
        const char* colp = cur + (64 * w + 2 * Lp) * 4 + kg * 8 * 1024;
#pragma unroll
        for (int kb = 0; kb < 4; ++kb) {
            floatx2 v[8];
#pragma unroll
            for (int e = 0; e < 8; ++e) v[e] = *reinterpret_cast<const floatx2*>(colp + (kb * 16 + e) * 1024) * HF_ASCALE;
            uintx4 bh[2], bl[2];
#pragma unroll
            for (int p = 0; p < 4; ++p) {
                unsigned h0, l0, h1, l1;
                split_pair(v[2 * p].x, v[2 * p + 1].x, h0, l0);
                split_pair(v[2 * p].y, v[2 * p + 1].y, h1, l1);
                bh[0][p] = h0; bl[0][p] = l0; bh[1][p] = h1; bl[1][p] = l1;
            }
#pragma unroll
            for (int rb = 0; rb < 2; ++rb)
#pragma unroll
                for (int f = 0; f < 2; ++f) acc[rb][f] = mfma_hh(A1[rb][kb][1], bh[f], acc[rb][f]);
#pragma unroll
            for (int rb = 0; rb < 2; ++rb)
#pragma unroll
                for (int f = 0; f < 2; ++f) acc[rb][f] = mfma_hh(A1[rb][kb][0], bl[f], acc[rb][f]);
#pragma unroll
            for (int rb = 0; rb < 2; ++rb)
#pragma unroll
                for (int f = 0; f < 2; ++f) acc[rb][f] = mfma_hh(A1[rb][kb][0], bh[f], acc[rb][f]);
        }

        if constexpr (MODE == G16_INV) {
            const float osc = 1.f / (F_SCALE * HF_ASCALE);
            const int kpg = tile32 * TILE + (w & 1) * 16 + (Lp >> 1);
            if (kpg < a.B) {
#pragma unroll
                for (int f = 0; f < 2; ++f) {
                    const int c = c8 * 8 + (w >> 1) * 4 + 2 * (Lp & 1) + f;
                    float* dst = a.out32 + ((size_t)kpg * F + c) * G;
#pragma unroll
                    for (int rb = 0; rb < 2; ++rb)
#pragma unroll
                        for (int t4 = 0; t4 < 4; ++t4) {
                            const int g0 = 32 * rb + 8 * t4 + 4 * kg;
                            floatx4 o;
                            o.x = acc[rb][f][4 * t4] * osc; o.y = acc[rb][f][4 * t4 + 1] * osc;
                            o.z = acc[rb][f][4 * t4 + 2] * osc; o.w = acc[rb][f][4 * t4 + 3] * osc;
                            if (g0 < G) *reinterpret_cast<floatx4*>(dst + g0) = o;
                        }
                }
            }
            continue;
        }

        if constexpr (MODE == G16_INVP || MODE == G16_INVG) {
            const int ch0 = c8 * 8 + (w >> 1) * 4 + 2 * (Lp & 1);
            const float d1 = 1.f / (F_SCALE * HF_ASCALE);
            const float s0 = a.bn_s[ch0] * d1 * H2_ASCALE, s1 = a.bn_s[ch0 + 1] * d1 * H2_ASCALE;
            const float t0 = a.bn_t[ch0] * H2_ASCALE, t1 = a.bn_t[ch0 + 1] * H2_ASCALE;
            const int kp = (w & 1) * 16 + (Lp >> 1);
            if (kg == 0) {
                floatx2 o;
                o.x = acc[0][0][0] * d1; o.y = acc[0][1][0] * d1;
                *reinterpret_cast<floatx2*>(a.res0 + (((((size_t)tile32 * a.C8 + c8) * G + 0) * 2 + (w >> 1)) * TILE + kp) * 4 + 2 * (Lp & 1)) = o;
            }
            __syncthreads();
            char* st = cur + (w >> 1) * 256 + kp * 8 + (Lp & 1) * 4;
#pragma unroll
            for (int rb = 0; rb < 2; ++rb)
#pragma unroll
                for (int r = 0; r < 16; ++r) {
                    const int g = 32 * rb + (r & 3) + 8 * (r >> 2) + 4 * kg;
                    unsigned hi, lo;
                    split_pair(fmaxf(acc[rb][0][r] * s0 + t0, 0.f), fmaxf(acc[rb][1][r] * s1 + t1, 0.f), hi, lo, top);
                    if (g < G) {
                        *reinterpret_cast<unsigned*>(st + g * 512) = hi;
                        *reinterpret_cast<unsigned*>(st + 30720 + g * 512) = lo;
                    }
                }
            __syncthreads();
            if constexpr (MODE == G16_INVG) {
                const int cb = c8 >> 2, sub = (c8 >> 1) & 1, kgr = c8 & 1, nslot = a.nTiles16, CB = a.C8 >> 2;
                char* dstg = a.planes + ((size_t)(tile32 >> 3) * nslot * CB + cb) * 32768 + ((sub * 2 + kgr) * 256 + (tile32 & 7) * 32) * 16;
#pragma unroll
                for (int i = 0; i < 15; ++i) {
                    const int idx = i * 256 + tid;
                    const int pl = idx >= 1920 ? 1 : 0, rem = idx - pl * 1920;
                    const int g = rem >> 5, kpp = rem & 31;
                    const int sl = qs[g];
                    const char* sp = cur + pl * 30720 + g * 512 + kpp * 8;
                    const uint2 c03 = *reinterpret_cast<const uint2*>(sp);
                    const uint2 c47 = *reinterpret_cast<const uint2*>(sp + 256);
                    if (sl >= 0) *reinterpret_cast<uintx4*>(dstg + (size_t)sl * CB * 32768 + pl * 16384 + kpp * 16) = uintx4{c03.x, c03.y, c47.x, c47.y};
                }
                continue;
            }
#pragma unroll
            for (int i = 0; i < 15; ++i) {
                const int idx = i * 256 + tid;
                const int pl = idx >= 1920 ? 1 : 0, rem = idx - pl * 1920;
                const int g = rem >> 5, kpp = rem & 31;
                const int t16 = 2 * tile32 + (kpp >> 4);
                const char* sp = cur + pl * 30720 + g * 512 + kpp * 8;
                const uint2 c03 = *reinterpret_cast<const uint2*>(sp);
                const uint2 c47 = *reinterpret_cast<const uint2*>(sp + 256);
                if (t16 < a.nTiles16)
                    *reinterpret_cast<uintx4*>(a.planes + (((size_t)t16 * a.C8 + c8) * 2 + pl) * 15360 + g * 256 + (kpp & 15) * 16) =
                        uintx4{c03.x, c03.y, c47.x, c47.y};
            }
            continue;
        }

        const int ch0 = c8 * 8 + (w >> 1) * 4 + 2 * (Lp & 1);
        const float dscale1 = 1.f / (F_SCALE * HF_ASCALE);
        const float s0 = a.bn_s[ch0] * dscale1 * H2_ASCALE, s1 = a.bn_s[ch0 + 1] * dscale1 * H2_ASCALE;
        const float t0 = a.bn_t[ch0] * H2_ASCALE, t1 = a.bn_t[ch0 + 1] * H2_ASCALE;
        floatx16 acc2[2][2];
#pragma unroll
        for (int rb = 0; rb < 2; ++rb)
#pragma unroll
            for (int f = 0; f < 2; ++f)
#pragma unroll
                for (int r = 0; r < 16; ++r) acc2[rb][f][r] = 0.f;
#pragma unroll
        for (int kb = 0; kb < 4; ++kb) {
            uintx4 bh[2], bl[2];
#pragma unroll
            for (int p = 0; p < 4; ++p) {
                const int r = 8 * (kb & 1) + 2 * p;
                const float y00 = fmaxf(acc[kb >> 1][0][r] * s0 + t0, 0.f), y01 = fmaxf(acc[kb >> 1][0][r + 1] * s0 + t0, 0.f);
                const float y10 = fmaxf(acc[kb >> 1][1][r] * s1 + t1, 0.f), y11 = fmaxf(acc[kb >> 1][1][r + 1] * s1 + t1, 0.f);
                unsigned h0, l0, h1, l1;
                split_pair(y00, y01, h0, l0);
                split_pair(y10, y11, h1, l1);
                bh[0][p] = h0; bl[0][p] = l0; bh[1][p] = h1; bl[1][p] = l1;
            }
#pragma unroll
            for (int rb = 0; rb < 2; ++rb)
#pragma unroll
                for (int f = 0; f < 2; ++f) acc2[rb][f] = mfma_hh(A2[rb][kb][1], bh[f], acc2[rb][f]);
#pragma unroll
            for (int rb = 0; rb < 2; ++rb)
#pragma unroll
                for (int f = 0; f < 2; ++f) acc2[rb][f] = mfma_hh(A2[rb][kb][0], bl[f], acc2[rb][f]);
#pragma unroll
            for (int rb = 0; rb < 2; ++rb)
#pragma unroll
                for (int f = 0; f < 2; ++f) acc2[rb][f] = mfma_hh(A2[rb][kb][0], bh[f], acc2[rb][f]);
        }

        if (PLANES) {
            const float osc = HF_ASCALE / (F_SCALE * H2_ASCALE);
            __syncthreads();
            const int kp = (w & 1) * 16 + (Lp >> 1);
            char* st = cur + (w >> 1) * 256 + kp * 8 + (Lp & 1) * 4;
#pragma unroll
            for (int rb = 0; rb < 2; ++rb)
#pragma unroll
                for (int r = 0; r < 16; ++r) {
                    const int q = 32 * rb + (r & 3) + 8 * (r >> 2) + 4 * kg;
                    unsigned hi, lo;
                    split_pair(acc2[rb][0][r] * osc, acc2[rb][1][r] * osc, hi, lo, top);
                    if (q < G) {
                        *reinterpret_cast<unsigned*>(st + q * 512) = hi;
                        *reinterpret_cast<unsigned*>(st + 30720 + q * 512) = lo;
                    }
                }
            __syncthreads();
            char* dst0 = a.planes + (size_t)(c8 >> 2) * 32768 + (c8 & 3) * 4096 + (tile32 & 7) * 512;
            const int nt = tile32 >> 3;
#pragma unroll
            for (int i = 0; i < 15; ++i) {
                const int idx = i * 256 + tid;
                const int pl = idx >= 1920 ? 1 : 0, rem = idx - pl * 1920;
                const int q = rem >> 5, kpp = rem & 31;
                const char* sp = cur + pl * 30720 + q * 512 + kpp * 8;
                const uint2 c03 = *reinterpret_cast<const uint2*>(sp);
                const uint2 c47 = *reinterpret_cast<const uint2*>(sp + 256);
                *reinterpret_cast<uintx4*>(dst0 + qb[q] + (long long)nt * qs[q] + kpp * 16 + pl * 16384) = uintx4{c03.x, c03.y, c47.x, c47.y};
            }
        } else {
            const float osc = 1.f / (F_SCALE * H2_ASCALE);
            float* dst = a.out32 + (size_t)chunk * CHUNK_FLOATS + 64 * w + 2 * Lp;
#pragma unroll
            for (int rb = 0; rb < 2; ++rb)
#pragma unroll
                for (int r = 0; r < 16; ++r) {
                    const int q = 32 * rb + (r & 3) + 8 * (r >> 2) + 4 * kg;
                    floatx2 o;
                    o.x = acc2[rb][0][r] * osc; o.y = acc2[rb][1][r] * osc;
                    if (q < G) *reinterpret_cast<floatx2*>(dst + q * 256) = o;
                }
        }
    }
    note_range_bits(a.rflag, top);
    if constexpr (MODE == G16_INVG) {
        if (a.amax) {
            unsigned m = top;
#pragma unroll
            for (int o = 32; o > 0; o >>= 1) m = max(m, (unsigned)__shfl_xor((int)m, o));
            if (lane == 0 && m) atomicMax(a.amax, m);
        }
    }
}

__device__ __forceinline__ unsigned half_of(float x) {
    const _Float16 h = (_Float16)x;
    unsigned short u;
    __builtin_memcpy(&u, &h, 2);
    return u;
}

__global__ __launch_bounds__(512, 2) void gft16x_kernel(Gft16Args a) {
    extern __shared__ __attribute__((aligned(16))) char smem[];
    const int tid = threadIdx.x, lane = tid & 63;
    const int w8 = __builtin_amdgcn_readfirstlane(tid >> 6);
    const int n = lane & 31, kg = lane >> 5;

    for (int i = tid; i < 2 * 256; i += 512) {
        const int bsel = i >> 8, j = i & 255;
        reinterpret_cast<uintx4*>(smem + bsel * GB + G * 1024)[j] = uintx4{0u, 0u, 0u, 0u};
    }
    long long* qb = reinterpret_cast<long long*>(smem + 2 * GB);
    int* qs = reinterpret_cast<int*>(smem + 2 * GB + 512);
    if (tid < G) { qb[tid] = a.qbase[tid]; qs[tid] = a.qstride[tid]; }
    float* bnl = reinterpret_cast<float*>(smem + G16_LDS);
    for (int i = tid; i < a.C8 * 8; i += 512) { bnl[i] = a.bn_s[i]; bnl[G16X_MAXC + i] = a.bn_t[i]; }

    uintx4 A1[2][4][2], A2[2][4][2];
#pragma unroll
    for (int rb = 0; rb < 2; ++rb)
#pragma unroll
        for (int kb = 0; kb < 4; ++kb)
#pragma unroll
            for (int pl = 0; pl < 2; ++pl) {
                A1[rb][kb][pl] = a.Ffrag[(((0 * 2 + rb) * 4 + kb) * 2 + pl) * 64 + lane];
                A2[rb][kb][pl] = a.Ffrag[(((1 * 2 + rb) * 4 + kb) * 2 + pl) * 64 + lane];
            }
    auto lds_barrier = [] {
        asm volatile("s_waitcnt lgkmcnt(0)" ::: "memory");
        __builtin_amdgcn_s_barrier();
        __builtin_amdgcn_sched_barrier(0);
    };
    auto stage = [&](int chunk, char* dst) {
        const int c8 = chunk % a.C8, tile32 = chunk / a.C8;
        const char* src = reinterpret_cast<const char*>(a.in) + ((size_t)tile32 * G * a.C8 + c8) * 1024;
        const size_t rs = (size_t)a.C8 * 1024;
#ifdef YOHO_EXPERIMENTS
        if (a.drain & 2) {
            for (int p = w8; p < G; p += 8) __builtin_amdgcn_global_load_lds((gptr_t)(src + p * rs + lane * 16), (lptr_t)(dst + p * 1024), 16, 0, 2);
            return;
        }
#endif
        for (int p = w8; p < G; p += 8) __builtin_amdgcn_global_load_lds((gptr_t)(src + p * rs + lane * 16), (lptr_t)(dst + p * 1024), 16, 0, 0);
    };
    const int hsel = w8 >> 2, kp = 8 * (w8 & 3) + (n >> 2), e = n & 3;
    unsigned top = 0u;
    int* ids = reinterpret_cast<int*>(smem + 2 * GB + 768);
    const bool steal = a.ctr != nullptr;
    int chunk = blockIdx.x, nxt = blockIdx.x + gridDim.x;
    int ticket = 0;
    if (steal) {
        if (tid == 0) {
            const int t0 = __hip_atomic_fetch_add(a.ctr, 2, __ATOMIC_RELAXED, __HIP_MEMORY_SCOPE_AGENT);
            ids[2] = t0;
        }
        __syncthreads();
        chunk = ids[2];
        nxt = chunk + 1;
    }
    if (chunk < a.nChunks) stage(chunk, smem);
    __builtin_amdgcn_s_waitcnt(0x0F70);
    for (int it = 0; chunk < a.nChunks; ++it) {
        char* cur = smem + (it & 1) * GB;
        if (it > 0) {
            if (a.drain & 1) asm volatile("s_waitcnt vmcnt(0)" ::: "memory");
            else if (w8 < 4) asm volatile("s_waitcnt vmcnt(8)" ::: "memory");
            else asm volatile("s_waitcnt vmcnt(7)" ::: "memory");
        }
        if (steal) {
            const unsigned emask = (unsigned)__builtin_amdgcn_readfirstlane(w8 == 0 ? 1 : 0);
            unsigned long long esave;
            asm volatile("s_mov_b64 %[sv], exec\n\t"
                         "s_mov_b32 exec_lo, %[m]\n\t"
                         "s_mov_b32 exec_hi, 0\n\t"
                         "ds_write_b32 %[slot], %[t]\n\t"
                         "global_atomic_add %[t], %[addr], %[one], off sc0\n\t"
                         "s_mov_b64 exec, %[sv]"
                         : [t] "+v"(ticket), [sv] "=&s"(esave)
                         : [m] "s"(emask), [slot] "v"((unsigned)(size_t)(ids + (it & 1))), [addr] "v"(a.ctr), [one] "v"(1)
                         : "memory");
        }
        lds_barrier();
        if (steal && it > 0) {
            int t;
            asm volatile("ds_read_b32 %0, %1\n\ts_waitcnt lgkmcnt(0)" : "=v"(t) : "v"((unsigned)(size_t)(ids + (it & 1))) : "memory");
            nxt = __builtin_amdgcn_readfirstlane(t);
        }
        const int next = nxt;
        if (next < a.nChunks) stage(next, smem + ((it + 1) & 1) * GB);
        const int c8 = chunk % a.C8, tile32 = chunk / a.C8;

        floatx16 acc[2];
#pragma unroll
        for (int rb = 0; rb < 2; ++rb)
#pragma unroll
            for (int r = 0; r < 16; ++r) acc[rb][r] = 0.f;
        const char* colp = cur + (32 * w8 + n) * 4 + kg * 8 * 1024;
#pragma unroll
        for (int kb = 0; kb < 4; ++kb) {
            float v[8];
#pragma unroll
            for (int i = 0; i < 8; ++i) v[i] = *reinterpret_cast<const float*>(colp + (kb * 16 + i) * 1024) * HF_ASCALE;
            uintx4 bh, bl;
#pragma unroll
            for (int p = 0; p < 4; ++p) {
                unsigned h, l;
                split_pair(v[2 * p], v[2 * p + 1], h, l);
                bh[p] = h; bl[p] = l;
            }
#pragma unroll
            for (int rb = 0; rb < 2; ++rb) acc[rb] = mfma_hh(A1[rb][kb][1], bh, acc[rb]);
#pragma unroll
            for (int rb = 0; rb < 2; ++rb) acc[rb] = mfma_hh(A1[rb][kb][0], bl, acc[rb]);
#pragma unroll
            for (int rb = 0; rb < 2; ++rb) acc[rb] = mfma_hh(A1[rb][kb][0], bh, acc[rb]);
        }
        const int ch = c8 * 8 + hsel * 4 + e;
        const float dscale1 = 1.f / (F_SCALE * HF_ASCALE);
        const float sc = bnl[ch] * dscale1 * H2_ASCALE, sh = bnl[G16X_MAXC + ch] * H2_ASCALE;
        floatx16 acc2[2];
#pragma unroll
        for (int rb = 0; rb < 2; ++rb)
#pragma unroll
            for (int r = 0; r < 16; ++r) acc2[rb][r] = 0.f;
#pragma unroll
        for (int kb = 0; kb < 4; ++kb) {
            uintx4 bh, bl;
#pragma unroll
            for (int p = 0; p < 4; ++p) {
                const int r = 8 * (kb & 1) + 2 * p;
                unsigned h, l;
                split_pair(fmaxf(acc[kb >> 1][r] * sc + sh, 0.f), fmaxf(acc[kb >> 1][r + 1] * sc + sh, 0.f), h, l);
                bh[p] = h; bl[p] = l;
            }
#pragma unroll
            for (int rb = 0; rb < 2; ++rb) acc2[rb] = mfma_hh(A2[rb][kb][1], bh, acc2[rb]);
#pragma unroll
            for (int rb = 0; rb < 2; ++rb) acc2[rb] = mfma_hh(A2[rb][kb][0], bl, acc2[rb]);
#pragma unroll
            for (int rb = 0; rb < 2; ++rb) acc2[rb] = mfma_hh(A2[rb][kb][0], bh, acc2[rb]);
        }
        const float osc = HF_ASCALE / (F_SCALE * H2_ASCALE);
        lds_barrier();
        char* st = cur + hsel * 256 + kp * 8 + e * 2;
#pragma unroll
        for (int rb = 0; rb < 2; ++rb)
#pragma unroll
            for (int r = 0; r < 16; ++r) {
                const int q = 32 * rb + (r & 3) + 8 * (r >> 2) + 4 * kg;
                const float x = acc2[rb][r] * osc;
                top = max(top, __float_as_uint(x) & 0x7FFFFFFFu);
                const _Float16 hh = (_Float16)x;
                if (q < G) {
                    *reinterpret_cast<unsigned short*>(st + q * 512) = (unsigned short)half_of(x);
                    *reinterpret_cast<unsigned short*>(st + 30720 + q * 512) = (unsigned short)half_of(x - (float)hh);
                }
            }
        lds_barrier();
        char* dst0 = a.planes + (size_t)(c8 >> 2) * 32768 + (c8 & 3) * 4096 + (tile32 & 7) * 512;
        const int nt = tile32 >> 3;
#pragma unroll
        for (int i = 0; i < 8; ++i) {
            const int idx = i * 512 + tid;
            if (idx < 2 * G * 32) {
                const int pl = idx >= 1920 ? 1 : 0, rem = idx - pl * 1920;
                const int q = rem >> 5, kpp = rem & 31;
                const char* sp = cur + pl * 30720 + q * 512 + kpp * 8;
                uint2 c03, c47;
                asm volatile("ds_read_b64 %0, %2\n\tds_read_b64 %1, %2 offset:256\n\ts_waitcnt lgkmcnt(0)"
                             : "=&v"(c03), "=&v"(c47) : "v"((unsigned)(size_t)sp) : "memory");
                *reinterpret_cast<uintx4*>(dst0 + qb[q] + (long long)nt * qs[q] + kpp * 16 + pl * 16384) = uintx4{c03.x, c03.y, c47.x, c47.y};
            }
        }
        chunk = next;
        if (!steal) nxt = next + gridDim.x;
    }
    note_range_bits(a.rflag, top);
    if (a.amax) {
        unsigned t = top;
#pragma unroll
        for (int o = 32; o >= 1; o >>= 1) t = max(t, (unsigned)__shfl_xor((int)t, o));
        if (lane == 0) atomicMax(a.amax, t);
    }
    if (steal && tid == 0) {
        __builtin_amdgcn_s_waitcnt(0x0F70);
        const int done = __hip_atomic_fetch_add(a.ctr + 1, 1, __ATOMIC_ACQ_REL, __HIP_MEMORY_SCOPE_AGENT);
        if (done == (int)gridDim.x - 1) {
            __hip_atomic_store(a.ctr, 0, __ATOMIC_RELAXED, __HIP_MEMORY_SCOPE_AGENT);
            __hip_atomic_store(a.ctr + 1, 0, __ATOMIC_RELEASE, __HIP_MEMORY_SCOPE_AGENT);
        }
    }
}

static inline unsigned short hbits(float x) {
    const _Float16 h = (_Float16)x;
    unsigned short u;
    std::memcpy(&u, &h, 2);
    return u;
}

void build_gft16_frags(const FourierBasis& fb, std::vector<unsigned short>& out) {
    out.assign((size_t)3 * 2 * 4 * 2 * 64 * 8, 0);
    auto Fv = [&](int q, int g) -> float { return (q < G && g < G) ? (float)fb.F[q * G + g] : 0.f; };
    for (int mat = 0; mat < 3; ++mat)
        for (int rb = 0; rb < 2; ++rb)
            for (int kb = 0; kb < 4; ++kb)
                for (int lane = 0; lane < 64; ++lane)
                    for (int e = 0; e < 8; ++e) {
                        const int i = lane & 31, kg = lane >> 5;
                        float v;
                        if (mat == 0) {
                            const int g = 32 * rb + i, q = 16 * kb + 8 * kg + e;
                            v = Fv(q, g);
                        } else if (mat == 1) {
                            const int q = 32 * rb + i;
                            const int g = 32 * (kb >> 1) + (e & 3) + 8 * (2 * (kb & 1) + (e >> 2)) + 4 * kg;
                            v = Fv(q, g);
                        } else {
                            const int q = 32 * rb + i, g = 16 * kb + 8 * kg + e;
                            v = Fv(q, g);
                        }
                        v *= F_SCALE;
                        const _Float16 hi = (_Float16)v;
                        const size_t base = ((((size_t)mat * 2 + rb) * 4 + kb) * 2) * 512 + lane * 8 + e;
                        out[base] = hbits(v);
                        out[base + 512] = hbits(v - (float)hi);
                    }
}

int gft16_init() {
    HIPCHK(hipFuncSetAttribute(reinterpret_cast<const void*>(&gft16_kernel<G16_ACT32>), hipFuncAttributeMaxDynamicSharedMemorySize, G16_LDS));
    HIPCHK(hipFuncSetAttribute(reinterpret_cast<const void*>(&gft16_kernel<G16_ACTP>), hipFuncAttributeMaxDynamicSharedMemorySize, G16_LDS));
    HIPCHK(hipFuncSetAttribute(reinterpret_cast<const void*>(&gft16_kernel<G16_INV>), hipFuncAttributeMaxDynamicSharedMemorySize, G16_LDS));
    HIPCHK(hipFuncSetAttribute(reinterpret_cast<const void*>(&gft16_kernel<G16_INVP>), hipFuncAttributeMaxDynamicSharedMemorySize, G16_LDS));
    HIPCHK(hipFuncSetAttribute(reinterpret_cast<const void*>(&gft16_kernel<G16_INVG>), hipFuncAttributeMaxDynamicSharedMemorySize, G16_LDS));
    HIPCHK(hipFuncSetAttribute(reinterpret_cast<const void*>(&gft16x_kernel), hipFuncAttributeMaxDynamicSharedMemorySize, G16X_LDS));
    return 0;
}

static void fill_qtables(int kppad, int cin, long long* qbase, int* qstride) {
    int qi[G * 4];
    long long off[NIR_ORD];
    fgemm_qinfo(qi);
    fgemm_plane_offsets(kppad, cin, off);
    for (int q = 0; q < G; ++q) {
        const int t = qi[q * 4], m = qi[q * 4 + 1], j = qi[q * 4 + 2], d = qi[q * 4 + 3];
        const long long KS = d * cin / 32;
        qstride[q] = (int)(KS * 32768);
        qbase[q] = off[t] + ((long long)j * (kppad / 256) * KS + (long long)m * cin / 32) * 32768;
    }
}

int launch_gft16(const float* in, float* out32, char* planes, int kppad, const void* Ffrag, const float* bn_s, const float* bn_t, int nTiles,
                 int C8, int nCU, hipStream_t s, int B, int* rflag, int variant, int* ctr, unsigned* amax) {
    Gft16Args a;
    a.B = B; a.res0 = nullptr; a.nTiles16 = 0; a.rflag = rflag; a.amax = amax;
    a.ctr = ctr;
    a.in = in; a.out32 = out32; a.planes = planes; a.Ffrag = reinterpret_cast<const uintx4*>(Ffrag); a.bn_s = bn_s; a.bn_t = bn_t;
    a.nChunks = nTiles * C8; a.C8 = C8;
    static const int dbg_drain = [] { const char* e = experiment_env("YOHO_PARTI_DEBUG"); return (e && std::strstr(e, "drain")) ? 1 : 0; }();
    static const int dbg_xf1 = [] { const char* e = experiment_env("YOHO_PARTI_DEBUG"); return (e && std::strstr(e, "xf1")) ? 1 : 0; }();
    static const int dbg_ldnt = [] { const char* e = experiment_env("YOHO_PARTI_DEBUG"); return (e && std::strstr(e, "ldnt")) ? 2 : 0; }();
    a.drain = dbg_drain | dbg_ldnt;
    if (dbg_xf1) variant = 1;
    if (planes) {
        fill_qtables(kppad, C8 * 8, a.qbase, a.qstride);
    } else {
        for (int q = 0; q < G; ++q) { a.qbase[q] = 0; a.qstride[q] = 0; }
    }
    static const int gmult = [] { const char* e = experiment_env("YOHO_PARTI_DEBUG"); const char* q = e ? std::strstr(e, "xfgrid") : nullptr; return q ? std::atoi(q + 6) : 1; }();
    const int want = nCU * (gmult > 0 ? gmult : 1);
    const int grid = a.nChunks < want ? a.nChunks : want;
    if (grid == 0) return 0;
    if (a.nChunks <= 2 * grid) a.ctr = nullptr;
    if (planes && variant != 1 && a.C8 * 8 <= G16X_MAXC) hipLaunchKernelGGL(gft16x_kernel, dim3(grid), dim3(512), G16X_LDS, s, a);
    else if (planes) hipLaunchKernelGGL(gft16_kernel<G16_ACTP>, dim3(grid), dim3(256), G16_LDS, s, a);
    else if (bn_s) hipLaunchKernelGGL(gft16_kernel<G16_ACT32>, dim3(grid), dim3(256), G16_LDS, s, a);
    else hipLaunchKernelGGL(gft16_kernel<G16_INV>, dim3(grid), dim3(256), G16_LDS, s, a);
    HIPCHK(hipGetLastError());
    return 0;
}

struct Head16Args {
    const float* x;
    const float* x1;
    int B0;
    char* planes;
    const uintx4* Ffrag;
    int B, nTiles;
    long long qbase[G];
    int qstride[G];
    int* rflag;
};

__global__ __launch_bounds__(256, 1) void head16_kernel(Head16Args a) {
    __shared__ long long qb[G];
    __shared__ int qs[G];
    const int tid = threadIdx.x, lane = tid & 63;
    const int w = __builtin_amdgcn_readfirstlane(tid >> 6);
    const int Lp = lane & 31, kg = lane >> 5;
    if (tid < G) { qb[tid] = a.qbase[tid]; qs[tid] = a.qstride[tid]; }
    __syncthreads();
    const int tile32 = blockIdx.x;
    const int kp = tile32 * TILE + Lp;
    unsigned top = 0u;
    uintx4 A[2][4][2];
#pragma unroll
    for (int rb = 0; rb < 2; ++rb)
#pragma unroll
        for (int kb = 0; kb < 4; ++kb)
#pragma unroll
            for (int pl = 0; pl < 2; ++pl) A[rb][kb][pl] = a.Ffrag[(((2 * 2 + rb) * 4 + kb) * 2 + pl) * 64 + lane];

    floatx16 acc[8][2];
#pragma unroll
    for (int f = 0; f < 8; ++f) {
#pragma unroll
        for (int rb = 0; rb < 2; ++rb)
#pragma unroll
            for (int r = 0; r < 16; ++r) acc[f][rb][r] = 0.f;
        const float* xrow = (a.x1 && kp >= a.B0) ? a.x1 + (size_t)(kp - a.B0) * (F * G) : a.x + (size_t)kp * (F * G);
        const float* xp = xrow + (size_t)(8 * w + f) * G + 8 * kg;
        floatx4 v[4][2];
#pragma unroll
        for (int kb = 0; kb < 4; ++kb) {
            const bool ok = kp < a.B;
            v[kb][0] = ok ? *reinterpret_cast<const floatx4*>(xp + 16 * kb) : floatx4{0.f, 0.f, 0.f, 0.f};
            v[kb][1] = (ok && (16 * kb + 8 * kg + 4) < G) ? *reinterpret_cast<const floatx4*>(xp + 16 * kb + 4) : floatx4{0.f, 0.f, 0.f, 0.f};
        }
#pragma unroll
        for (int kb = 0; kb < 4; ++kb) {
            uintx4 bh, bl;
            unsigned h, l;
            split_pair(v[kb][0].x * H2_ASCALE, v[kb][0].y * H2_ASCALE, h, l); bh.x = h; bl.x = l;
            split_pair(v[kb][0].z * H2_ASCALE, v[kb][0].w * H2_ASCALE, h, l); bh.y = h; bl.y = l;
            split_pair(v[kb][1].x * H2_ASCALE, v[kb][1].y * H2_ASCALE, h, l); bh.z = h; bl.z = l;
            split_pair(v[kb][1].z * H2_ASCALE, v[kb][1].w * H2_ASCALE, h, l); bh.w = h; bl.w = l;
#pragma unroll
            for (int rb = 0; rb < 2; ++rb) acc[f][rb] = mfma_hh(A[rb][kb][1], bh, acc[f][rb]);
#pragma unroll
            for (int rb = 0; rb < 2; ++rb) acc[f][rb] = mfma_hh(A[rb][kb][0], bl, acc[f][rb]);
#pragma unroll
            for (int rb = 0; rb < 2; ++rb) acc[f][rb] = mfma_hh(A[rb][kb][0], bh, acc[f][rb]);
        }
    }
    const float osc = HF_ASCALE / (F_SCALE * H2_ASCALE);
    char* dst0 = a.planes + (w & 3) * 4096 + ((tile32 & 7) * 32 + Lp) * 16;
    const int nt = tile32 >> 3;
#pragma unroll
    for (int rb = 0; rb < 2; ++rb)
#pragma unroll
        for (int r = 0; r < 16; ++r) {
            const int q = 32 * rb + (r & 3) + 8 * (r >> 2) + 4 * kg;
            uintx4 ph, pl;
            unsigned h, l;
            split_pair(acc[0][rb][r] * osc, acc[1][rb][r] * osc, h, l, top); ph.x = h; pl.x = l;
            split_pair(acc[2][rb][r] * osc, acc[3][rb][r] * osc, h, l, top); ph.y = h; pl.y = l;
            split_pair(acc[4][rb][r] * osc, acc[5][rb][r] * osc, h, l, top); ph.z = h; pl.z = l;
            split_pair(acc[6][rb][r] * osc, acc[7][rb][r] * osc, h, l, top); ph.w = h; pl.w = l;
            if (q < G) {
                char* d = dst0 + qb[q] + (long long)nt * qs[q];
                *reinterpret_cast<uintx4*>(d) = ph;
                *reinterpret_cast<uintx4*>(d + 16384) = pl;
            }
        }
    note_range_bits(a.rflag, top);
}

int launch_head16(const float* x, int B, int nTiles, char* planes, int kppad, const void* Ffrag, hipStream_t s, const float* x1, int B0,
                  int* rflag) {
    Head16Args a;
    a.rflag = rflag;
    a.x = x; a.x1 = x1; a.B0 = B0; a.planes = planes; a.Ffrag = reinterpret_cast<const uintx4*>(Ffrag); a.B = B; a.nTiles = nTiles;
    fill_qtables(kppad, 32, a.qbase, a.qstride);
    if (nTiles == 0) return 0;
    hipLaunchKernelGGL(head16_kernel, dim3(nTiles), dim3(256), 0, s, a);
    HIPCHK(hipGetLastError());
    return 0;
}

int launch_gft16_invp(const float* in, float* res0, char* planes16, int nTiles16, const void* Ffrag, const float* bn_s, const float* bn_t,
                      int nTiles, int C8, int nCU, hipStream_t s, int* rflag) {
    Gft16Args a;
    a.rflag = rflag; a.drain = 0; a.ctr = nullptr; a.amax = nullptr;
    a.in = in; a.out32 = nullptr; a.planes = planes16; a.Ffrag = reinterpret_cast<const uintx4*>(Ffrag); a.bn_s = bn_s; a.bn_t = bn_t;
    a.nChunks = nTiles * C8; a.C8 = C8; a.B = 0; a.res0 = res0; a.nTiles16 = nTiles16;
    for (int q = 0; q < G; ++q) { a.qbase[q] = 0; a.qstride[q] = 0; }
    const int grid = a.nChunks < nCU ? a.nChunks : nCU;
    if (grid == 0) return 0;
    hipLaunchKernelGGL(gft16_kernel<G16_INVP>, dim3(grid), dim3(256), G16_LDS, s, a);
    HIPCHK(hipGetLastError());
    return 0;
}

int launch_gft16_invg(const float* in, float* res0, char* planesG, const int* slot_of, int nslot, const void* Ffrag, const float* bn_s,
                      const float* bn_t, int nTiles, int C8, int nCU, hipStream_t s, int* rflag, unsigned* amax) {
    Gft16Args a;
    a.rflag = rflag; a.drain = 0; a.ctr = nullptr; a.amax = amax;
    a.in = in; a.out32 = nullptr; a.planes = planesG; a.Ffrag = reinterpret_cast<const uintx4*>(Ffrag); a.bn_s = bn_s; a.bn_t = bn_t;
    a.nChunks = nTiles * C8; a.C8 = C8; a.B = 0; a.res0 = res0; a.nTiles16 = nslot;
    for (int q = 0; q < G; ++q) { a.qbase[q] = 0; a.qstride[q] = slot_of[q]; }
    const int grid = a.nChunks < nCU ? a.nChunks : nCU;
    if (grid == 0) return 0;
    hipLaunchKernelGGL(gft16_kernel<G16_INVG>, dim3(grid), dim3(256), G16_LDS, s, a);
    HIPCHK(hipGetLastError());
    return 0;
}

struct Head2Args {
    const float* src[4];
    const int64_t* ridx[4];
    int istride;
    const int64_t* pre_idx;
    const int* P;
    const float* bn_s;
    const float* bn_t;
    char* planes;
    const uintx4* Ffrag;
    int M;
    long long qbase[G];
    int qstride[G];
    int* rflag;
};

constexpr int H2_STG = 8192;

__global__ __launch_bounds__(256, 1) void head2_kernel(Head2Args a) {
    __shared__ long long qb[G];
    __shared__ int qs[G];
    __shared__ __attribute__((aligned(16))) char stg[4][2][H2_STG];
    const int tid = threadIdx.x, lane = tid & 63;
    const int w = __builtin_amdgcn_readfirstlane(tid >> 6);
    const int Lp = lane & 31, kg = lane >> 5;
    if (tid < G) { qb[tid] = a.qbase[tid]; qs[tid] = a.qstride[tid]; }
    __syncthreads();
    const int tile32 = blockIdx.x;
    const int sidx = blockIdx.y;
    const int m = tile32 * TILE + Lp;
    const bool ok = m < a.M;
    unsigned top = 0u;
    uintx4 A[2][4][2];
#pragma unroll
    for (int rb = 0; rb < 2; ++rb)
#pragma unroll
        for (int kb = 0; kb < 4; ++kb)
#pragma unroll
            for (int pl = 0; pl < 2; ++pl) A[rb][kb][pl] = a.Ffrag[(((2 * 2 + rb) * 4 + kb) * 2 + pl) * 64 + lane];
    int gsrc[4][8];
    {
        long long pi = ok ? a.pre_idx[m] : 0;
        pi = pi < 0 ? 0 : (pi > 59 ? 59 : pi);
#pragma unroll
        for (int kb = 0; kb < 4; ++kb)
#pragma unroll
            for (int e = 0; e < 8; ++e) {
                const int gp = 16 * kb + 8 * kg + e;
                gsrc[kb][e] = gp < G ? a.P[(int)pi * G + gp] : 0;
            }
    }
    const int nt = tile32 >> 3;
    const float osc = HF_ASCALE / (F_SCALE * H2_ASCALE);
    {
        const int cblk = sidx * 4 + w;
        const size_t srow = (ok && a.ridx[sidx]) ? (size_t)a.ridx[sidx][(size_t)m * a.istride] : (size_t)m;
        const float* sp = a.src[sidx] + srow * (F * G) + (size_t)(w * 8) * G;
        const bool permute = (sidx == 0) || (sidx == 2);
        int rowj[8];
        const int dl = lane < 60 ? lane : lane - 15;
        const int dmi = dl / 15, dpc = dl - dmi * 15;
        if (permute) {
#pragma unroll
            for (int j = 0; j < 8; ++j) {
                int mm = tile32 * TILE + 4 * j + dmi;
                mm = mm < a.M ? mm : a.M - 1;
                rowj[j] = a.ridx[sidx] ? (int)a.ridx[sidx][(size_t)mm * a.istride] : mm;
            }
        }
        auto stage = [&](int f, int buf) {
            const char* base = reinterpret_cast<const char*>(a.src[sidx]) + (size_t)(w * 8 + f) * (G * 4) + dpc * 16;
#pragma unroll
            for (int j = 0; j < 8; ++j)
                __builtin_amdgcn_global_load_lds((gptr_t)(base + (size_t)rowj[j] * (F * G * 4)), (lptr_t)(&stg[w][buf][j * 1024]), 16, 0, 0);
        };
        if (permute) stage(0, 0);
        const char* myrow = &stg[w][0][(Lp >> 2) * 1024 + (Lp & 3) * 240];
        floatx16 acc[8][2];
#pragma unroll
        for (int f = 0; f < 8; ++f) {
#pragma unroll
            for (int rb = 0; rb < 2; ++rb)
#pragma unroll
                for (int r = 0; r < 16; ++r) acc[f][rb][r] = 0.f;
            const float bs = a.bn_s[cblk * 8 + f] * H2_ASCALE, bt = a.bn_t[cblk * 8 + f] * H2_ASCALE;
            const float* xp = sp + f * G;
            float v[4][8];
            if (permute) {
                const char* rowf = myrow + (f & 1) * H2_STG;
#pragma unroll
                for (int kb = 0; kb < 4; ++kb)
#pragma unroll
                    for (int e = 0; e < 8; ++e) {
                        const float t = *reinterpret_cast<const float*>(rowf + gsrc[kb][e] * 4);
                        v[kb][e] = ok ? t : 0.f;
                    }
                if (f + 1 < 8) {
                    asm volatile("s_waitcnt lgkmcnt(0)" ::: "memory");
                    stage(f + 1, (f + 1) & 1);
                }
            } else {
#pragma unroll
                for (int kb = 0; kb < 4; ++kb) {
                    const floatx4 lo4 = ok ? *reinterpret_cast<const floatx4*>(xp + 16 * kb + 8 * kg) : floatx4{0.f, 0.f, 0.f, 0.f};
                    const floatx4 hi4 = (ok && (16 * kb + 8 * kg + 4) < G) ? *reinterpret_cast<const floatx4*>(xp + 16 * kb + 8 * kg + 4)
                                                                           : floatx4{0.f, 0.f, 0.f, 0.f};
                    v[kb][0] = lo4.x; v[kb][1] = lo4.y; v[kb][2] = lo4.z; v[kb][3] = lo4.w;
                    v[kb][4] = hi4.x; v[kb][5] = hi4.y; v[kb][6] = hi4.z; v[kb][7] = hi4.w;
                }
            }
#pragma unroll
            for (int kb = 0; kb < 4; ++kb) {
                uintx4 bh, bl;
#pragma unroll
                for (int p = 0; p < 4; ++p) {
                    const bool v0 = ok && (16 * kb + 8 * kg + 2 * p) < G, v1 = ok && (16 * kb + 8 * kg + 2 * p + 1) < G;
                    const float y0 = v0 ? fmaxf(v[kb][2 * p] * bs + bt, 0.f) : 0.f;
                    const float y1 = v1 ? fmaxf(v[kb][2 * p + 1] * bs + bt, 0.f) : 0.f;
                    unsigned h, l;
                    split_pair(y0, y1, h, l);
                    bh[p] = h; bl[p] = l;
                }
#pragma unroll
                for (int rb = 0; rb < 2; ++rb) acc[f][rb] = mfma_hh(A[rb][kb][1], bh, acc[f][rb]);
#pragma unroll
                for (int rb = 0; rb < 2; ++rb) acc[f][rb] = mfma_hh(A[rb][kb][0], bl, acc[f][rb]);
#pragma unroll
                for (int rb = 0; rb < 2; ++rb) acc[f][rb] = mfma_hh(A[rb][kb][0], bh, acc[f][rb]);
            }
        }
        char* dst0 = a.planes + (size_t)(cblk >> 2) * 32768 + (cblk & 3) * 4096 + ((tile32 & 7) * 32 + Lp) * 16;
#pragma unroll
        for (int rb = 0; rb < 2; ++rb)
#pragma unroll
            for (int r = 0; r < 16; ++r) {
                const int q = 32 * rb + (r & 3) + 8 * (r >> 2) + 4 * kg;
                uintx4 ph, pl;
                unsigned h, l;
                split_pair(acc[0][rb][r] * osc, acc[1][rb][r] * osc, h, l, top); ph.x = h; pl.x = l;
                split_pair(acc[2][rb][r] * osc, acc[3][rb][r] * osc, h, l, top); ph.y = h; pl.y = l;
                split_pair(acc[4][rb][r] * osc, acc[5][rb][r] * osc, h, l, top); ph.z = h; pl.z = l;
                split_pair(acc[6][rb][r] * osc, acc[7][rb][r] * osc, h, l, top); ph.w = h; pl.w = l;
                if (q < G) {
                    char* d = dst0 + qb[q] + (long long)nt * qs[q];
                    *reinterpret_cast<uintx4*>(d) = ph;
                    *reinterpret_cast<uintx4*>(d + 16384) = pl;
                }
            }
    }
    note_range_bits(a.rflag, top);
}

int launch_head2(const float* s0, const float* s1, const float* s2, const float* s3, const int64_t* pre_idx, const int* P, const float* bn_s,
                 const float* bn_t, int M, int nTiles, char* planes, int kppad, const void* Ffrag, hipStream_t s, const int64_t* const* ridx,
                 int istride, int* rflag) {
    Head2Args a;
    a.rflag = rflag;
    a.src[0] = s0; a.src[1] = s1; a.src[2] = s2; a.src[3] = s3;
    for (int i = 0; i < 4; ++i) a.ridx[i] = ridx ? ridx[i] : nullptr;
    a.istride = istride;
    a.pre_idx = pre_idx; a.P = P; a.bn_s = bn_s; a.bn_t = bn_t; a.planes = planes; a.Ffrag = reinterpret_cast<const uintx4*>(Ffrag); a.M = M;
    fill_qtables(kppad, 128, a.qbase, a.qstride);
    if (nTiles == 0) return 0;
    hipLaunchKernelGGL(head2_kernel, dim3(nTiles, 4), dim3(256), 0, s, a);
    HIPCHK(hipGetLastError());
    return 0;
}

}
```

Baseline: 1.935 million keypoints/s.

## Pack irrep column blocks contiguously instead of padding each to kppad

Replaces the per-irrep keypoint padding (each j block padded to kppad) with a packed column layout where column units are (j, tile32) pairs indexed j*nT32+tile32, so N-tiles are computed from d*nT32 rather than d*kppad. The plane writers (head16, head2, gft16) now compute per-q base offsets from a unit index, and the epilogues map unit indices back to (j, tile32). A host-side search also picks XCD rotation offsets per irrep order to balance cost across the 8 XCDs. This removes padded GEMM work and tiles, at the price of more index arithmetic and a 32-keypoint tile granularity for column blocks.

```diff
diff --git a/yoho_amd/csrc/gemmf.h b/yoho_amd/csrc/gemmf.h
--- a/yoho_amd/csrc/gemmf.h
+++ b/yoho_amd/csrc/gemmf.h
@@ -29,7 +29,7 @@
     long long a_off[NIR_ORD], b_off[NIR_ORD];
     int NT[NIR_ORD], MT[NIR_ORD], rot[NIR_ORD];
     int dim[NIR_ORD], qbase[NIR_ORD];
-    int cin, cout, kppad, nT32;
+    int cin, cout, nT32;
     float descale;
     int* rflag;
     const unsigned* amax;
@@ -65,7 +65,7 @@
             for (int e = 0; e < 16; ++e) acc[i][j][e] = 0.f;
 }
 
-__device__ __forceinline__ bool fg3_map(const FGemmArgs& a, int xcd, int slot, int& t, int& local, int& r) {
+__host__ __device__ __forceinline__ bool fg3_map(const FGemmArgs& a, int xcd, int slot, int& t, int& local, int& r) {
     int start = 0;
     for (int u = 0; u < NIR_ORD; ++u) {
         const int ru = (xcd + a.rot[u]) & 7;
@@ -74,6 +74,63 @@
         start += cnt;
     }
     return false;
+}
+
+__host__ __device__ __forceinline__ void col_unit(int u, int nT32, int& j, int& tile32) {
+    j = u / nT32;
+    tile32 = u - j * nT32;
+}
+
+inline void fgemm_fill_map(FGemmArgs& a, int cin, int cout, int nT32) {
+    a.cin = cin; a.cout = cout; a.nT32 = nT32;
+    int cost[NIR_ORD][8], cnt[NIR_ORD][8];
+    for (int t = 0; t < NIR_ORD; ++t) {
+        a.MT[t] = (FG_ORD_D[t] * cout + 255) / 256;
+        a.NT[t] = (FG_ORD_D[t] * nT32 + 7) / 8;
+        a.dim[t] = FG_ORD_D[t];
+        a.qbase[t] = FG_IR_BASE[FG_ORD_R[t]];
+        for (int r = 0; r < 8; ++r) {
+            cnt[t][r] = a.NT[t] > r ? ((a.NT[t] - 1 - r) / 8 + 1) * a.MT[t] : 0;
+            cost[t][r] = cnt[t][r] * FG_ORD_D[t];
+        }
+    }
+    struct Lists { int cost[8], cnt[8]; };
+    auto add = [&](const Lists& l, int t, int r) {
+        Lists o;
+        for (int x = 0; x < 8; ++x) { o.cost[x] = l.cost[x] + cost[t][(x + r) & 7]; o.cnt[x] = l.cnt[x] + cnt[t][(x + r) & 7]; }
+        return o;
+    };
+    auto better = [](const Lists& l, int& worst, int& grid) {
+        int w = 0, g = 0;
+        for (int x = 0; x < 8; ++x) { w = l.cost[x] > w ? l.cost[x] : w; g = l.cnt[x] > g ? l.cnt[x] : g; }
+        if (w > worst || (w == worst && g >= grid)) return false;
+        worst = w; grid = g;
+        return true;
+    };
+    const Lists none = {};
+    const int ROT[NIR_ORD] = {0, 0, 4, 4, 2};
+    Lists l = none;
+    for (int t = 0; t < 4; ++t) l = add(l, t, ROT[t]);
+    int worst = 0x7FFFFFFF, grid = 0x7FFFFFFF;
+    (void)better(l, worst, grid);
+    Lists l4 = l;
+    for (int t = 0; t < 4; ++t) a.rot[t] = ROT[t];
+    const Lists l0 = add(none, 0, 0);
+    for (int r1 = 0; r1 < 8; ++r1) {
+        const Lists l1 = add(l0, 1, r1);
+        for (int r2 = 0; r2 < 8; ++r2) {
+            const Lists l2 = add(l1, 2, r2);
+            for (int r3 = 0; r3 < 8; ++r3) {
+                const Lists l3 = add(l2, 3, r3);
+                if (better(l3, worst, grid)) { a.rot[1] = r1; a.rot[2] = r2; a.rot[3] = r3; l4 = l3; }
+            }
+        }
+    }
+    worst = grid = 0x7FFFFFFF;
+    a.rot[4] = ROT[4];
+    (void)better(add(l4, 4, ROT[4]), worst, grid);
+    for (int r4 = 0; r4 < 8; ++r4)
+        if (better(add(l4, 4, r4), worst, grid)) a.rot[4] = r4;
 }
 
 inline int fgemm_grid(const FGemmArgs& a, int per_tile) {
@@ -96,18 +153,19 @@
 }
 
 template <int MI, int NJ>
-__device__ __forceinline__ void residual_start(floatx16 (&acc)[MI][NJ], int row0, int kp0, int jidx, int d, int qbase, const float* res, float descale,
+__device__ __forceinline__ void residual_start(floatx16 (&acc)[MI][NJ], int row0, int u0, int d, int qbase, const float* res, float descale,
                                                int cout, int nT32, int lane) {
     const float inv = 1.f / descale;
     const int half = lane >> 5, kp32 = lane & 31, cout8 = cout >> 3;
 #pragma unroll
     for (int bi = 0; bi < NJ; ++bi) {
-        const int tile32 = (kp0 >> 5) + bi;
+        int jidx, tile32;
+        col_unit(u0 + bi, nT32, jidx, tile32);
 #pragma unroll
         for (int ai = 0; ai < MI; ++ai) {
             const int rowb = row0 + ai * 32;
             const int iidx = rowb / cout, o0 = rowb - iidx * cout;
-            const bool ok = tile32 < nT32 && iidx < d;
+            const bool ok = jidx < d && iidx < d;
             const int q = qbase + iidx * d + jidx;
 #pragma unroll
             for (int q4 = 0; q4 < 4; ++q4) {
@@ -121,7 +179,7 @@
 }
 
 template <int MI, int NJ>
-__device__ __forceinline__ void coef_epilogue(const floatx16 (&acc)[MI][NJ], int row0, int kp0, int jidx, int d, int qbase, float* out, const float* bias,
+__device__ __forceinline__ void coef_epilogue(const floatx16 (&acc)[MI][NJ], int row0, int u0, int d, int qbase, float* out, const float* bias,
                                               float descale, int cout, int nT32, int* rflag, int lane, int flags) {
     const int half = lane >> 5, kp32 = lane & 31, cout8 = cout >> 3;
     unsigned top = 0u;
@@ -132,8 +190,9 @@
 #endif
 #pragma unroll
     for (int bi = 0; bi < NJ; ++bi) {
-        const int tile32 = (kp0 >> 5) + bi;
-        if (tile32 >= nT32) continue;
+        int jidx, tile32;
+        col_unit(u0 + bi, nT32, jidx, tile32);
+        if (jidx >= d) continue;
 #pragma unroll
         for (int ai = 0; ai < MI; ++ai) {
             const int rowb = row0 + ai * 32;
@@ -229,19 +288,20 @@
 }
 
 template <int MI, int NJ>
-__device__ __forceinline__ void residual_start(floatx4 (&acc)[MI][NJ], int row0, int kp0, int jidx, int d, int qbase, const float* res, float descale,
+__device__ __forceinline__ void residual_start(floatx4 (&acc)[MI][NJ], int row0, int u0, int d, int qbase, const float* res, float descale,
                                                int cout, int nT32, int lane) {
     static_assert(NJ % 2 == 0, "pairs of 16-column tiles");
     const float inv = 1.f / descale;
     const int half = lane >> 5, kp32 = lane & 31, cout8 = cout >> 3;
 #pragma unroll
     for (int bi = 0; bi < NJ; bi += 2) {
-        const int tile32 = (kp0 >> 5) + (bi >> 1);
+        int jidx, tile32;
+        col_unit(u0 + (bi >> 1), nT32, jidx, tile32);
 #pragma unroll
         for (int ai = 0; ai < MI; ++ai) {
             const int rowb = row0 + ai * 16;
             const int iidx = rowb / cout, o0 = rowb - iidx * cout;
-            const bool ok = tile32 < nT32 && iidx < d;
+            const bool ok = jidx < d && iidx < d;
             const int q = qbase + iidx * d + jidx;
             const size_t off0 = slab_off(tile32, q, cout8, o0 + half * 4, half, kp32), off1 = slab_off(tile32, q, cout8, o0 + 8 + half * 4, half, kp32);
             acc[ai][bi] = *reinterpret_cast<const floatx4*>(res + (ok ? off0 : 0)) * (ok ? inv : 0.f);
@@ -252,15 +312,16 @@
 }
 
 template <int MI, int NJ>
-__device__ __forceinline__ void coef_epilogue(const floatx4 (&acc)[MI][NJ], int row0, int kp0, int jidx, int d, int qbase, float* out, const float* bias,
+__device__ __forceinline__ void coef_epilogue(const floatx4 (&acc)[MI][NJ], int row0, int u0, int d, int qbase, float* out, const float* bias,
                                               float descale, int cout, int nT32, int* rflag, int lane, int flags) {
     static_assert(NJ % 2 == 0, "pairs of 16-column tiles");
     const int half = lane >> 5, kp32 = lane & 31, cout8 = cout >> 3;
     unsigned top = 0u;
 #pragma unroll
     for (int bi = 0; bi < NJ; bi += 2) {
-        const int tile32 = (kp0 >> 5) + (bi >> 1);
-        if (tile32 >= nT32) continue;
+        int jidx, tile32;
+        col_unit(u0 + (bi >> 1), nT32, jidx, tile32);
+        if (jidx >= d) continue;
 #pragma unroll
         for (int ai = 0; ai < MI; ++ai) {
             const int rowb = row0 + ai * 16;
diff --git a/yoho_amd/csrc/gemmf.hip b/yoho_amd/csrc/gemmf.hip
--- a/yoho_amd/csrc/gemmf.hip
+++ b/yoho_amd/csrc/gemmf.hip
@@ -100,7 +100,7 @@
         stage_tile(Ag + FG_STAGE, smem + 2 * FG_STAGE, w, lane);
         stage_tile(Bg + FG_STAGE, smem + 3 * FG_STAGE, w, lane);
     }
-    if ((flags & EPI_RES) && row0 < d * a.cout) residual_start(acc, row0, col0 % a.kppad, col0 / a.kppad, d, a.qbase[t], a.res, a.descale, a.cout, a.nT32, lane);
+    if ((flags & EPI_RES) && row0 < d * a.cout) residual_start(acc, row0, col0 >> 5, d, a.qbase[t], a.res, a.descale, a.cout, a.nT32, lane);
     asm volatile("s_waitcnt vmcnt(0)" ::: "memory");
     __syncthreads();
 
@@ -131,7 +131,7 @@
     }
     asm volatile("s_waitcnt vmcnt(0)" ::: "memory");
 
-    coef_epilogue(acc, row0, col0 % a.kppad, col0 / a.kppad, d, a.qbase[t], a.out, a.bias, a.descale, a.cout, a.nT32, a.rflag, lane, flags);
+    coef_epilogue(acc, row0, col0 >> 5, d, a.qbase[t], a.out, a.bias, a.descale, a.cout, a.nT32, a.rflag, lane, flags);
 }
 
 __global__ __launch_bounds__(256, 1) void fgemmk_kernel(FGemmArgs a, int flags) {
@@ -160,7 +160,7 @@
         stage_tile(Ag + FG_STAGE, smem + 2 * FG_STAGE, w, lane);
         stage_tile(Bg + FG_STAGE, smem + 3 * FG_STAGE, w, lane);
     }
-    if ((flags & EPI_RES) && rows_live) residual_start(acc, row0, col0 % a.kppad, col0 / a.kppad, d, a.qbase[t], a.res, a.descale, a.cout, a.nT32, lane);
+    if ((flags & EPI_RES) && rows_live) residual_start(acc, row0, col0 >> 5, d, a.qbase[t], a.res, a.descale, a.cout, a.nT32, lane);
     asm volatile("s_waitcnt vmcnt(0)" ::: "memory");
     __syncthreads();
     for (int s = 0; s < KS; ++s) {
@@ -174,7 +174,7 @@
             stage_tile(uniform_ptr(Bg + (size_t)(s + 2) * FG_STAGE), cur + FG_STAGE, w, lane);
         }
     }
-    if (rows_live) coef_epilogue(acc, row0, col0 % a.kppad, col0 / a.kppad, d, a.qbase[t], a.out, a.bias, a.descale, a.cout, a.nT32, a.rflag, lane, flags);
+    if (rows_live) coef_epilogue(acc, row0, col0 >> 5, d, a.qbase[t], a.out, a.bias, a.descale, a.cout, a.nT32, a.rflag, lane, flags);
 }
 
 int fgemm_init() {
@@ -320,16 +320,11 @@
 void fgemm_fill_args(FGemmArgs& a, const Layer& L, const char* Bplanes, int kppad, int nT32, const float* res, float* out, int* rflag) {
     a.rflag = rflag; a.amax = nullptr;
     a.A = reinterpret_cast<const char*>(L.wpg); a.B = Bplanes; a.bias = L.bias; a.res = res; a.out = out;
-    a.cin = L.cin; a.cout = L.cout; a.kppad = kppad; a.nT32 = nT32; a.descale = L.wpg_descale;
-    static const int ROT[NIR_ORD] = {0, 0, 4, 4, 2};
+    a.descale = L.wpg_descale;
+    fgemm_fill_map(a, L.cin, L.cout, nT32);
     for (int t = 0; t < NIR_ORD; ++t) {
         a.a_off[t] = pack_off(t, L.cout, L.cin);
         a.b_off[t] = pack_off(t, kppad, L.cin);
-        a.MT[t] = (FG_ORD_D[t] * L.cout + 255) / 256;
-        a.NT[t] = FG_ORD_D[t] * kppad / 256;
-        a.rot[t] = ROT[t];
-        a.dim[t] = FG_ORD_D[t];
-        a.qbase[t] = FG_IR_BASE[FG_ORD_R[t]];
     }
 }
 
diff --git a/yoho_amd/csrc/gemmf2.hip b/yoho_amd/csrc/gemmf2.hip
--- a/yoho_amd/csrc/gemmf2.hip
+++ b/yoho_amd/csrc/gemmf2.hip
@@ -185,8 +185,8 @@
     ring_prologue<F2_BUF>(KT, dma);
     const int row0 = mtile * 256 + wm * 128, colbase = ntile * 256 + nh * 128 + wn * 64;
     const bool rows_live = row0 < d * a.cout;
-    const int jidx = colbase / a.kppad, kp0 = colbase - jidx * a.kppad, qbase = a.qbase[t];
-    if ((flags & EPI_RES) && rows_live) residual_start(acc, row0, kp0, jidx, d, qbase, a.res, a.descale, a.cout, a.nT32, lane);
+    const int u0 = colbase >> 5, qbase = a.qbase[t];
+    if ((flags & EPI_RES) && rows_live) residual_start(acc, row0, u0, d, qbase, a.res, a.descale, a.cout, a.nT32, lane);
     asm volatile("s_waitcnt vmcnt(0)" ::: "memory");
     __builtin_amdgcn_s_barrier();
     if (!rows_live) return ring_pipelined_idle<F2_BUF>(KT, dma);
@@ -197,7 +197,7 @@
         [&](auto dmac, const Frags2& f, Frags2& nf, const char* ra, const char* rb, const char* srcA, const char* srcB, char* buf) {
             step2<decltype(dmac)::value>(dm, f, acc, ra, rb, nf, srcA, srcB, buf);
         });
-    coef_epilogue(acc, row0, kp0, jidx, d, qbase, a.out, a.bias, a.descale, a.cout, a.nT32, a.rflag, lane, flags);
+    coef_epilogue(acc, row0, u0, d, qbase, a.out, a.bias, a.descale, a.cout, a.nT32, a.rflag, lane, flags);
 }
 
 struct Wave3 {
@@ -228,8 +228,8 @@
     ring_prologue<F3_BUF>(KT, dma);
     const int row0 = mtile * 256 + wv.wm * 128, colbase = ntile * 256 + wv.nh * 128 + wv.wn * 64;
     const bool rows_live = row0 < d * a.cout;
-    const int jidx = colbase / a.kppad, kp0 = colbase - jidx * a.kppad, qbase = a.qbase[t];
-    if ((flags & EPI_RES) && rows_live) residual_start(acc, row0, kp0, jidx, d, qbase, a.res, a.descale, a.cout, a.nT32, lane);
+    const int u0 = colbase >> 5, qbase = a.qbase[t];
+    if ((flags & EPI_RES) && rows_live) residual_start(acc, row0, u0, d, qbase, a.res, a.descale, a.cout, a.nT32, lane);
     asm volatile("s_waitcnt vmcnt(0)" ::: "memory");
     __builtin_amdgcn_s_barrier();
     if (!rows_live) return ring_pipelined_idle<F3_BUF>(KT, dma);
@@ -240,7 +240,7 @@
         [&](auto dmac, const Frags2& f, Frags2& nf, const char* ra, const char* rb, const char* srcA, const char* srcB, char* buf) {
             step2<decltype(dmac)::value>(wv.dm, f, acc, ra, rb, nf, srcA, srcB, buf);
         });
-    coef_epilogue(acc, row0, kp0, jidx, d, qbase, a.out, a.bias, a.descale, a.cout, a.nT32, a.rflag, lane, flags);
+    coef_epilogue(acc, row0, u0, d, qbase, a.out, a.bias, a.descale, a.cout, a.nT32, a.rflag, lane, flags);
 }
 
 constexpr int F3K_BUF = 2 * FG_STAGE;
@@ -320,8 +320,8 @@
     if (KS > 1) dma(1, F3K_BUF);
     const int row0 = mtile * 256 + wm * 128, colbase = ntile * 256 + nh * 128 + wn * 64;
     const bool rows_live = row0 < d * a.cout;
-    const int jidx = colbase / a.kppad, kp0 = colbase - jidx * a.kppad, qbase = a.qbase[t];
-    if ((flags & EPI_RES) && rows_live) residual_start(acc, row0, kp0, jidx, d, qbase, a.res, a.descale, a.cout, a.nT32, lane);
+    const int u0 = colbase >> 5, qbase = a.qbase[t];
+    if ((flags & EPI_RES) && rows_live) residual_start(acc, row0, u0, d, qbase, a.res, a.descale, a.cout, a.nT32, lane);
     asm volatile("s_waitcnt vmcnt(0)" ::: "memory");
     __builtin_amdgcn_s_barrier();
     if (!rows_live) {
@@ -355,7 +355,7 @@
     }
     run(dman, P, Q);
     run(dman, Q, P);
-    coef_epilogue(acc, row0, kp0, jidx, d, qbase, a.out, a.bias, a.descale, a.cout, a.nT32, a.rflag, lane, flags);
+    coef_epilogue(acc, row0, u0, d, qbase, a.out, a.bias, a.descale, a.cout, a.nT32, a.rflag, lane, flags);
 }
 
 constexpr int F2K_BUF = FG_STAGE + FG_STAGE / 2;
@@ -395,8 +395,8 @@
     if (KS > 1) dma(1, F2K_BUF);
     const int row0 = mtile * 256 + wm * 128, colbase = ntile * 256 + nh * 128 + wn * 64;
     const bool rows_live = row0 < d * a.cout;
-    const int jidx = colbase / a.kppad, kp0 = colbase - jidx * a.kppad, qbase = a.qbase[t];
-    if ((flags & EPI_RES) && rows_live) residual_start(acc, row0, kp0, jidx, d, qbase, a.res, a.descale, a.cout, a.nT32, lane);
+    const int u0 = colbase >> 5, qbase = a.qbase[t];
+    if ((flags & EPI_RES) && rows_live) residual_start(acc, row0, u0, d, qbase, a.res, a.descale, a.cout, a.nT32, lane);
     asm volatile("s_waitcnt vmcnt(0)" ::: "memory");
     __builtin_amdgcn_s_barrier();
     for (int s = 0; s < KS; ++s) {
@@ -407,7 +407,7 @@
         __builtin_amdgcn_sched_barrier(0);
         if (s + 2 < KS) dma(s + 2, cur);
     }
-    if (rows_live) coef_epilogue(acc, row0, kp0, jidx, d, qbase, a.out, a.bias, a.descale, a.cout, a.nT32, a.rflag, lane, flags);
+    if (rows_live) coef_epilogue(acc, row0, u0, d, qbase, a.out, a.bias, a.descale, a.cout, a.nT32, a.rflag, lane, flags);
 }
 
 typedef int intx8 __attribute__((ext_vector_type(8)));
@@ -548,13 +548,13 @@
     dma_step(wv.dm, Ag + step_off(1), Bg + step_off(1), smem + F3_BUF);
     const int row0 = mtile * 256 + wv.wm * 128, colbase = ntile * 256 + wv.nh * 128 + wv.wn * 64;
     const bool rows_live = row0 < d * a.cout;
-    const int jidx = colbase / a.kppad, kp0 = colbase - jidx * a.kppad, qbase = a.qbase[t];
-    if ((flags & EPI_RES) && rows_live) residual_start(acc, row0, kp0, jidx, d, qbase, a.res, a.descale, a.cout, a.nT32, lane);
+    const int u0 = colbase >> 5, qbase = a.qbase[t];
+    if ((flags & EPI_RES) && rows_live) residual_start(acc, row0, u0, d, qbase, a.res, a.descale, a.cout, a.nT32, lane);
     asm volatile("s_waitcnt vmcnt(0)" ::: "memory");
     __builtin_amdgcn_s_barrier();
 
     ring_plain<true>(acc, smem, wv, Ag, [&](int s) { return Bg + step_off(s); }, KT, rows_live, sc);
-    if (rows_live) coef_epilogue(acc, row0, kp0, jidx, d, qbase, a.out, a.bias, a.descale, a.cout, a.nT32, a.rflag, lane, flags);
+    if (rows_live) coef_epilogue(acc, row0, u0, d, qbase, a.out, a.bias, a.descale, a.cout, a.nT32, a.rflag, lane, flags);
 }
 
 struct CGemmArgs {
@@ -850,8 +850,7 @@
         default: fgemm3s_kloop<5>(acc, smem, Ag, Bg, KT, dm, lane_a, lane_b); break;
     }
     const int colbase = ntile * 256 + w8 * 32;
-    const int jidx = colbase / a.kppad, kp0 = colbase - jidx * a.kppad;
-    coef_epilogue(acc, 0, kp0, jidx, d, a.qbase[t], a.out, a.bias, a.descale, 32, a.nT32, a.rflag, lane, flags & F2_NOSTORE);
+    coef_epilogue(acc, 0, colbase >> 5, d, a.qbase[t], a.out, a.bias, a.descale, 32, a.nT32, a.rflag, lane, flags & F2_NOSTORE);
 }
 
 int fgemm3_init() {
diff --git a/yoho_amd/csrc/gft16.hip b/yoho_amd/csrc/gft16.hip
--- a/yoho_amd/csrc/gft16.hip
+++ b/yoho_amd/csrc/gft16.hip
@@ -19,7 +19,7 @@
 typedef __attribute__((address_space(3))) void* lptr_t;
 
 constexpr int GB = 65536;
-constexpr int G16_LDS = 2 * GB + 1024;
+constexpr int G16_LDS = 2 * GB + 1536;
 constexpr int G16X_MAXC = 512;
 constexpr int G16X_LDS = G16_LDS + 2 * G16X_MAXC * 4;
 constexpr float F_SCALE = 1024.f;
@@ -36,6 +36,7 @@
     int nTiles16;
     long long qbase[G];
     int qstride[G];
+    int qunit[G];
     int* rflag;
     int drain;
     int* ctr;
@@ -69,6 +70,11 @@
     for (int p = w; p < G; p += 4) __builtin_amdgcn_global_load_lds((gptr_t)(s + p * rs + lane * 16), (lptr_t)(dst + p * 1024), 16, 0, 0);
 }
 
+__device__ __forceinline__ long long plane_base(long long qbase, int qstride, int qunit, int tile32) {
+    const int u = qunit + tile32;
+    return qbase + (long long)(u >> 3) * qstride + (u & 7) * 512;
+}
+
 enum { G16_ACT32 = 0, G16_ACTP = 1, G16_INV = 2, G16_INVP = 3, G16_INVG = 4 };
 
 template <int MODE>
@@ -85,7 +91,9 @@
     }
     long long* qb = reinterpret_cast<long long*>(smem + 2 * GB);
     int* qs = reinterpret_cast<int*>(smem + 2 * GB + 512);
-    if (tid < G) { qb[tid] = a.qbase[tid]; qs[tid] = a.qstride[tid]; }
+    int* qu = reinterpret_cast<int*>(smem + 2 * GB + 784);
+    long long* qo = reinterpret_cast<long long*>(smem + 2 * GB + 1024);
+    if (tid < G) { qb[tid] = a.qbase[tid]; qs[tid] = a.qstride[tid]; qu[tid] = a.qunit[tid]; }
 
     uintx4 A1[2][4][2], A2[2][4][2];
 #pragma unroll
@@ -280,9 +288,9 @@
                         *reinterpret_cast<unsigned*>(st + 30720 + q * 512) = lo;
                     }
                 }
+            if (tid < G) qo[tid] = plane_base(qb[tid], qs[tid], qu[tid], tile32);
             __syncthreads();
-            char* dst0 = a.planes + (size_t)(c8 >> 2) * 32768 + (c8 & 3) * 4096 + (tile32 & 7) * 512;
-            const int nt = tile32 >> 3;
+            char* dst0 = a.planes + (size_t)(c8 >> 2) * 32768 + (c8 & 3) * 4096;
 #pragma unroll
             for (int i = 0; i < 15; ++i) {
                 const int idx = i * 256 + tid;
@@ -291,7 +299,7 @@
                 const char* sp = cur + pl * 30720 + q * 512 + kpp * 8;
                 const uint2 c03 = *reinterpret_cast<const uint2*>(sp);
                 const uint2 c47 = *reinterpret_cast<const uint2*>(sp + 256);
-                *reinterpret_cast<uintx4*>(dst0 + qb[q] + (long long)nt * qs[q] + kpp * 16 + pl * 16384) = uintx4{c03.x, c03.y, c47.x, c47.y};
+                *reinterpret_cast<uintx4*>(dst0 + qo[q] + kpp * 16 + pl * 16384) = uintx4{c03.x, c03.y, c47.x, c47.y};
             }
         } else {
             const float osc = 1.f / (F_SCALE * H2_ASCALE);
@@ -337,7 +345,9 @@
     }
     long long* qb = reinterpret_cast<long long*>(smem + 2 * GB);
     int* qs = reinterpret_cast<int*>(smem + 2 * GB + 512);
-    if (tid < G) { qb[tid] = a.qbase[tid]; qs[tid] = a.qstride[tid]; }
+    int* qu = reinterpret_cast<int*>(smem + 2 * GB + 784);
+    long long* qo = reinterpret_cast<long long*>(smem + 2 * GB + 1024);
+    if (tid < G) { qb[tid] = a.qbase[tid]; qs[tid] = a.qstride[tid]; qu[tid] = a.qunit[tid]; }
     float* bnl = reinterpret_cast<float*>(smem + G16_LDS);
     for (int i = tid; i < a.C8 * 8; i += 512) { bnl[i] = a.bn_s[i]; bnl[G16X_MAXC + i] = a.bn_t[i]; }
 
@@ -481,9 +491,9 @@
                     *reinterpret_cast<unsigned short*>(st + 30720 + q * 512) = (unsigned short)half_of(x - (float)hh);
                 }
             }
+        if (tid < G) qo[tid] = plane_base(qb[tid], qs[tid], qu[tid], tile32);
         lds_barrier();
-        char* dst0 = a.planes + (size_t)(c8 >> 2) * 32768 + (c8 & 3) * 4096 + (tile32 & 7) * 512;
-        const int nt = tile32 >> 3;
+        char* dst0 = a.planes + (size_t)(c8 >> 2) * 32768 + (c8 & 3) * 4096;
 #pragma unroll
         for (int i = 0; i < 8; ++i) {
             const int idx = i * 512 + tid;
@@ -494,7 +504,7 @@
                 uint2 c03, c47;
                 asm volatile("ds_read_b64 %0, %2\n\tds_read_b64 %1, %2 offset:256\n\ts_waitcnt lgkmcnt(0)"
                              : "=&v"(c03), "=&v"(c47) : "v"((unsigned)(size_t)sp) : "memory");
-                *reinterpret_cast<uintx4*>(dst0 + qb[q] + (long long)nt * qs[q] + kpp * 16 + pl * 16384) = uintx4{c03.x, c03.y, c47.x, c47.y};
+                *reinterpret_cast<uintx4*>(dst0 + qo[q] + kpp * 16 + pl * 16384) = uintx4{c03.x, c03.y, c47.x, c47.y};
             }
         }
         chunk = next;
@@ -563,7 +573,7 @@
     return 0;
 }
 
-static void fill_qtables(int kppad, int cin, long long* qbase, int* qstride) {
+static void fill_qtables(int kppad, int nT32, int cin, long long* qbase, int* qstride, int* qunit) {
     int qi[G * 4];
     long long off[NIR_ORD];
     fgemm_qinfo(qi);
@@ -572,7 +582,8 @@
         const int t = qi[q * 4], m = qi[q * 4 + 1], j = qi[q * 4 + 2], d = qi[q * 4 + 3];
         const long long KS = d * cin / 32;
         qstride[q] = (int)(KS * 32768);
-        qbase[q] = off[t] + ((long long)j * (kppad / 256) * KS + (long long)m * cin / 32) * 32768;
+        qbase[q] = off[t] + ((long long)m * cin / 32) * 32768;
+        qunit[q] = j * nT32;
     }
 }
 
@@ -589,9 +600,9 @@
     a.drain = dbg_drain | dbg_ldnt;
     if (dbg_xf1) variant = 1;
     if (planes) {
-        fill_qtables(kppad, C8 * 8, a.qbase, a.qstride);
+        fill_qtables(kppad, nTiles, C8 * 8, a.qbase, a.qstride, a.qunit);
     } else {
-        for (int q = 0; q < G; ++q) { a.qbase[q] = 0; a.qstride[q] = 0; }
+        for (int q = 0; q < G; ++q) { a.qbase[q] = 0; a.qstride[q] = 0; a.qunit[q] = 0; }
     }
     static const int gmult = [] { const char* e = experiment_env("YOHO_PARTI_DEBUG"); const char* q = e ? std::strstr(e, "xfgrid") : nullptr; return q ? std::atoi(q + 6) : 1; }();
     const int want = nCU * (gmult > 0 ? gmult : 1);
@@ -615,18 +626,18 @@
     int B, nTiles;
     long long qbase[G];
     int qstride[G];
+    int qunit[G];
     int* rflag;
 };
 
 __global__ __launch_bounds__(256, 1) void head16_kernel(Head16Args a) {
-    __shared__ long long qb[G];
-    __shared__ int qs[G];
+    __shared__ long long qo[G];
     const int tid = threadIdx.x, lane = tid & 63;
     const int w = __builtin_amdgcn_readfirstlane(tid >> 6);
     const int Lp = lane & 31, kg = lane >> 5;
-    if (tid < G) { qb[tid] = a.qbase[tid]; qs[tid] = a.qstride[tid]; }
+    const int tile32 = blockIdx.x;
+    if (tid < G) qo[tid] = plane_base(a.qbase[tid], a.qstride[tid], a.qunit[tid], tile32);
     __syncthreads();
-    const int tile32 = blockIdx.x;
     const int kp = tile32 * TILE + Lp;
     unsigned top = 0u;
     uintx4 A[2][4][2];
@@ -670,8 +681,7 @@
         }
     }
     const float osc = HF_ASCALE / (F_SCALE * H2_ASCALE);
-    char* dst0 = a.planes + (w & 3) * 4096 + ((tile32 & 7) * 32 + Lp) * 16;
-    const int nt = tile32 >> 3;
+    char* dst0 = a.planes + (w & 3) * 4096 + Lp * 16;
 #pragma unroll
     for (int rb = 0; rb < 2; ++rb)
 #pragma unroll
@@ -684,7 +694,7 @@
             split_pair(acc[4][rb][r] * osc, acc[5][rb][r] * osc, h, l, top); ph.z = h; pl.z = l;
             split_pair(acc[6][rb][r] * osc, acc[7][rb][r] * osc, h, l, top); ph.w = h; pl.w = l;
             if (q < G) {
-                char* d = dst0 + qb[q] + (long long)nt * qs[q];
+                char* d = dst0 + qo[q];
                 *reinterpret_cast<uintx4*>(d) = ph;
                 *reinterpret_cast<uintx4*>(d + 16384) = pl;
             }
@@ -697,7 +707,7 @@
     Head16Args a;
     a.rflag = rflag;
     a.x = x; a.x1 = x1; a.B0 = B0; a.planes = planes; a.Ffrag = reinterpret_cast<const uintx4*>(Ffrag); a.B = B; a.nTiles = nTiles;
-    fill_qtables(kppad, 32, a.qbase, a.qstride);
+    fill_qtables(kppad, nTiles, 32, a.qbase, a.qstride, a.qunit);
     if (nTiles == 0) return 0;
     hipLaunchKernelGGL(head16_kernel, dim3(nTiles), dim3(256), 0, s, a);
     HIPCHK(hipGetLastError());
@@ -710,7 +720,7 @@
     a.rflag = rflag; a.drain = 0; a.ctr = nullptr; a.amax = nullptr;
     a.in = in; a.out32 = nullptr; a.planes = planes16; a.Ffrag = reinterpret_cast<const uintx4*>(Ffrag); a.bn_s = bn_s; a.bn_t = bn_t;
     a.nChunks = nTiles * C8; a.C8 = C8; a.B = 0; a.res0 = res0; a.nTiles16 = nTiles16;
-    for (int q = 0; q < G; ++q) { a.qbase[q] = 0; a.qstride[q] = 0; }
+    for (int q = 0; q < G; ++q) { a.qbase[q] = 0; a.qstride[q] = 0; a.qunit[q] = 0; }
     const int grid = a.nChunks < nCU ? a.nChunks : nCU;
     if (grid == 0) return 0;
     hipLaunchKernelGGL(gft16_kernel<G16_INVP>, dim3(grid), dim3(256), G16_LDS, s, a);
@@ -724,7 +734,7 @@
     a.rflag = rflag; a.drain = 0; a.ctr = nullptr; a.amax = amax;
     a.in = in; a.out32 = nullptr; a.planes = planesG; a.Ffrag = reinterpret_cast<const uintx4*>(Ffrag); a.bn_s = bn_s; a.bn_t = bn_t;
     a.nChunks = nTiles * C8; a.C8 = C8; a.B = 0; a.res0 = res0; a.nTiles16 = nslot;
-    for (int q = 0; q < G; ++q) { a.qbase[q] = 0; a.qstride[q] = slot_of[q]; }
+    for (int q = 0; q < G; ++q) { a.qbase[q] = 0; a.qstride[q] = slot_of[q]; a.qunit[q] = 0; }
     const int grid = a.nChunks < nCU ? a.nChunks : nCU;
     if (grid == 0) return 0;
     hipLaunchKernelGGL(gft16_kernel<G16_INVG>, dim3(grid), dim3(256), G16_LDS, s, a);
@@ -745,21 +755,21 @@
     int M;
     long long qbase[G];
     int qstride[G];
+    int qunit[G];
     int* rflag;
 };
 
 constexpr int H2_STG = 8192;
 
 __global__ __launch_bounds__(256, 1) void head2_kernel(Head2Args a) {
-    __shared__ long long qb[G];
-    __shared__ int qs[G];
+    __shared__ long long qo[G];
     __shared__ __attribute__((aligned(16))) char stg[4][2][H2_STG];
     const int tid = threadIdx.x, lane = tid & 63;
     const int w = __builtin_amdgcn_readfirstlane(tid >> 6);
     const int Lp = lane & 31, kg = lane >> 5;
-    if (tid < G) { qb[tid] = a.qbase[tid]; qs[tid] = a.qstride[tid]; }
+    const int tile32 = blockIdx.x;
+    if (tid < G) qo[tid] = plane_base(a.qbase[tid], a.qstride[tid], a.qunit[tid], tile32);
     __syncthreads();
-    const int tile32 = blockIdx.x;
     const int sidx = blockIdx.y;
     const int m = tile32 * TILE + Lp;
     const bool ok = m < a.M;
@@ -783,7 +793,6 @@
                 gsrc[kb][e] = gp < G ? a.P[(int)pi * G + gp] : 0;
             }
     }
-    const int nt = tile32 >> 3;
     const float osc = HF_ASCALE / (F_SCALE * H2_ASCALE);
     {
         const int cblk = sidx * 4 + w;
@@ -862,7 +871,7 @@
                 for (int rb = 0; rb < 2; ++rb) acc[f][rb] = mfma_hh(A[rb][kb][0], bh, acc[f][rb]);
             }
         }
-        char* dst0 = a.planes + (size_t)(cblk >> 2) * 32768 + (cblk & 3) * 4096 + ((tile32 & 7) * 32 + Lp) * 16;
+        char* dst0 = a.planes + (size_t)(cblk >> 2) * 32768 + (cblk & 3) * 4096 + Lp * 16;
 #pragma unroll
         for (int rb = 0; rb < 2; ++rb)
 #pragma unroll
@@ -875,7 +884,7 @@
                 split_pair(acc[4][rb][r] * osc, acc[5][rb][r] * osc, h, l, top); ph.z = h; pl.z = l;
                 split_pair(acc[6][rb][r] * osc, acc[7][rb][r] * osc, h, l, top); ph.w = h; pl.w = l;
                 if (q < G) {
-                    char* d = dst0 + qb[q] + (long long)nt * qs[q];
+                    char* d = dst0 + qo[q];
                     *reinterpret_cast<uintx4*>(d) = ph;
                     *reinterpret_cast<uintx4*>(d + 16384) = pl;
                 }
@@ -893,7 +902,7 @@
     for (int i = 0; i < 4; ++i) a.ridx[i] = ridx ? ridx[i] : nullptr;
     a.istride = istride;
     a.pre_idx = pre_idx; a.P = P; a.bn_s = bn_s; a.bn_t = bn_t; a.planes = planes; a.Ffrag = reinterpret_cast<const uintx4*>(Ffrag); a.M = M;
-    fill_qtables(kppad, 128, a.qbase, a.qstride);
+    fill_qtables(kppad, nTiles, 128, a.qbase, a.qstride, a.qunit);
     if (nTiles == 0) return 0;
     hipLaunchKernelGGL(head2_kernel, dim3(nTiles, 4), dim3(256), 0, s, a);
     HIPCHK(hipGetLastError());
```

Result: no change. 1.953 million keypoints/s (median of 6 runs) (+0.9%).
